# noah-aviel-dove/signals

Hardware: AMD Instinct MI355X
Metric: rendered Msamples/s (48 kHz, 256-sample blocks) (higher is better)
Workload: dtype f64; 1 GPU; C2: 1024-voice Fixed->Sine->LowPass->Gain->SumBus(stereo) per GPU, 48 kHz, 256-frame blocks, 4096 blocks per batch (f32 storage, f64 phase/recurrence); engine schedule = fused voice chain + bus: sig_fused_voice_bus (Sine->LowPass->Gain->SumBus in ONE launch, its voice tiles added in fixed order by the same kernel; no per-voice sample touches HBM); voices_per_gpu=1024, block_frames=256, start_position=0, parallelism=voices sharded 1024/GPU x1; single process, no collective, rccl_ranks=0

## Files before the change

### include/signals_amd.h

```cpp
#ifndef SIGNALS_AMD_H
#define SIGNALS_AMD_H

#include <stdint.h>

#ifdef __cplusplus
extern "C" {
#endif

#define SIG_ABI_VERSION 7

enum { SIG_F32 = 0, SIG_F64 = 1 };

enum { SIG_OSC_SINE = 0, SIG_OSC_SQUARE = 1, SIG_OSC_SAWTOOTH = 2, SIG_OSC_TRIANGLE = 3 };

enum { SIG_FILT_LOWPASS = 0, SIG_FILT_HIGHPASS = 1, SIG_FILT_BANDPASS = 2, SIG_FILT_BANDSTOP = 3 };

enum { SIG_EW_GAIN = 0, SIG_EW_MIX = 1, SIG_EW_RINGMOD = 2, SIG_EW_AMP = 3 };

enum { SIG_STATUS_BAD_CUTOFF = 1 };

int sig_abi_version(void);

int sig_osc_bank(int kind, int64_t position, int32_t rate, int64_t rows, int32_t voices,
                 const double* hertz, int32_t hertz_stride,
// ... 79 lines not shown

int sig_mix_matrix(int64_t rows, int32_t voices, const float* x, int64_t x_ld,
                   const float* matrix, float* out, int64_t out_ld, void* stream);

int sig_fused_osc_biquad(int osc_kind, int filt_type, int32_t rate, int64_t position,
                         int32_t block_frames, int32_t nblocks, int32_t context, int32_t voices,
                         const double* hertz, int32_t hertz_stride, const double* phase, int32_t phase_stride,
                         const double* cutoff, int32_t cutoff_stride,
                         const double* gain, int32_t gain_stride,
                         float* out, int64_t out_ld, int32_t* status, void* stream);

int sig_fused_osc_biquad_rows(int osc_kind, int filt_type, int32_t rate, int64_t position,
                              int32_t block_frames, int32_t nblocks, int32_t context, int32_t voices,
                              const double* hertz, int32_t hertz_stride, const double* phase, int32_t phase_stride,
                              const double* cutoff, int32_t cutoff_stride, int32_t cutoff_rows,
                              const double* gain, int32_t gain_stride, int32_t gain_rows,
                              float* out, int64_t out_ld, int32_t* status, void* stream);
int sig_fused_voice_bus_rows(int osc_kind, int filt_type, int32_t rate, int64_t position,
                             int32_t block_frames, int32_t nblocks, int32_t context, int32_t voices,
                             const double* hertz, int32_t hertz_stride, const double* phase, int32_t phase_stride,
                             const double* cutoff, int32_t cutoff_stride, int32_t cutoff_rows,
                             const double* gain, int32_t gain_stride, int32_t gain_rows,
                             const double* bus_gains, int64_t bus_gains_ld, int32_t bus_channels,
                             double* workspace, float* out, int64_t out_ld, int32_t* status, void* stream);

int sig_fused_osc_biquad_fm(int osc_kind, int filt_type, int32_t rate, int64_t position,
                            int32_t block_frames, int32_t nblocks, int32_t context, int32_t voices,
                            const double* hertz, int32_t hertz_stride, int32_t hertz_rows, const double* hertz_hist,
                            const double* phase, int32_t phase_stride, int32_t phase_rows, const double* phase_hist,
                            const double* cutoff, int32_t cutoff_stride, int32_t cutoff_rows,
                            const double* gain, int32_t gain_stride, int32_t gain_rows,
                            float* out, int64_t out_ld, int32_t* status, void* stream);
int sig_fused_voice_bus_fm(int osc_kind, int filt_type, int32_t rate, int64_t position,
                           int32_t block_frames, int32_t nblocks, int32_t context, int32_t voices,
                           const double* hertz, int32_t hertz_stride, int32_t hertz_rows, const double* hertz_hist,
                           const double* phase, int32_t phase_stride, int32_t phase_rows, const double* phase_hist,
                           const double* cutoff, int32_t cutoff_stride, int32_t cutoff_rows,
                           const double* gain, int32_t gain_stride, int32_t gain_rows,
                           const double* bus_gains, int64_t bus_gains_ld, int32_t bus_channels,
                           double* workspace, float* out, int64_t out_ld, int32_t* status, void* stream);

int sig_fused_osc_pair_biquad(int osc_kind, int osc2_kind, int pair_op, int filt_type, int32_t rate, int64_t position,
                              int32_t block_frames, int32_t nblocks, int32_t context, int32_t voices,
                              const double* hertz, int32_t hertz_stride, const double* phase, int32_t phase_stride,
                              const double* hertz2, int32_t hertz2_stride, const double* phase2, int32_t phase2_stride,
                              const double* mix, int32_t mix_stride,
                              const double* cutoff, int32_t cutoff_stride, int32_t cutoff_rows,
                              const double* gain, int32_t gain_stride, int32_t gain_rows,
                              float* out, int64_t out_ld, int32_t* status, void* stream);
int sig_fused_voice_pair_bus(int osc_kind, int osc2_kind, int pair_op, int filt_type, int32_t rate, int64_t position,
                             int32_t block_frames, int32_t nblocks, int32_t context, int32_t voices,
                             const double* hertz, int32_t hertz_stride, const double* phase, int32_t phase_stride,
                             const double* hertz2, int32_t hertz2_stride, const double* phase2, int32_t phase2_stride,
                             const double* mix, int32_t mix_stride,
                             const double* cutoff, int32_t cutoff_stride, int32_t cutoff_rows,
                             const double* gain, int32_t gain_stride, int32_t gain_rows,
                             const double* bus_gains, int64_t bus_gains_ld, int32_t bus_channels,
                             double* workspace, float* out, int64_t out_ld, int32_t* status, void* stream);

int sig_fused_osc_biquad_devpos(int osc_kind, int filt_type, int32_t rate, const int64_t* position_dev,
                                int32_t block_frames, int32_t nblocks, int32_t context, int32_t voices,
                                const double* hertz, int32_t hertz_stride, const double* phase, int32_t phase_stride,
                                const double* cutoff, int32_t cutoff_stride,
                                const double* gain, int32_t gain_stride,
                                float* out, int64_t out_ld, int32_t* status, void* stream);
int sig_advance_position(int64_t* position_dev, int64_t delta, void* stream);

enum { SIG_CTL_ROW = 0, SIG_CTL_OSC = 1, SIG_CTL_GAIN = 2, SIG_CTL_MIX = 3, SIG_CTL_RINGMOD = 4, SIG_CTL_AMP = 5,
       SIG_CTL_NOISE = 6, SIG_CTL_FILTER = 7 };
enum { SIG_CTL_MAX_REGS = 48, SIG_CTL_MAX_INS = 48 };
typedef struct {
    int32_t op;
    int32_t kind;
    int32_t a, b, c;
    int32_t dst;
    int32_t stride, rows;
    int32_t cols;
    int32_t reserved;
    const double* row;
} sig_ctl_ins;
typedef struct { int32_t reg; int32_t cols; double* out; double* front; } sig_ctl_out;
int sig_control_program(int32_t rate, int64_t position, int32_t step, int32_t nblocks, int32_t cols, int64_t front_position,
                        int64_t min_position,
                        const sig_ctl_ins* program, int32_t n_ins, const sig_ctl_out* outs, int32_t n_outs, void* stream);
int sig_control_program_windowed(int32_t rate, int64_t position, int32_t step, int32_t nblocks, int32_t cols, int64_t front_position,
                                 int64_t min_position,
                                 const sig_ctl_ins* program, int32_t n_ins, const sig_ctl_out* outs, int32_t n_outs, void* stream);

int sig_control_program_attach(const int32_t* description, int32_t n_words, const void* image, int32_t* handle);
int sig_control_program_attached(int32_t handle, int32_t rate, int64_t position, int32_t step, int32_t nblocks, int32_t cols,
                                 int64_t front_position, int64_t min_position,
                                 const sig_ctl_ins* program, int32_t n_ins, const sig_ctl_out* outs, int32_t n_outs, void* stream);

int sig_fused_osc_biquad_mix(int osc_kind, int filt_type, int32_t rate, int64_t position,
                             int32_t block_frames, int32_t nblocks, int32_t context, int32_t voices,
                             const double* hertz, int32_t hertz_stride, const double* phase, int32_t phase_stride,
                             const double* cutoff, int32_t cutoff_stride,
                             const double* gain, int32_t gain_stride,
                             const float* matrix, float* out, int64_t out_ld, int32_t* status, void* stream);

int64_t sig_fused_voice_bus_workspace(int32_t voices, int64_t rows, int32_t bus_channels);
int sig_fused_voice_bus_walk(int osc_kind, int filt_type, int32_t rate, int64_t position,
                             int32_t block_frames, int32_t nblocks, int32_t context, int32_t voices,
                             const double* hertz, int32_t hertz_stride, const double* phase, int32_t phase_stride,
                             const double* cutoff, int32_t cutoff_stride,
                             const double* gain, int32_t gain_stride,
                             const double* bus_gains, int64_t bus_gains_ld, int32_t bus_channels,
                             double* workspace, float* out, int64_t out_ld, int32_t* status, void* stream);
int64_t sig_fused_voice_consts_size(int32_t voices);
int sig_fused_voice_bus_prepared(int osc_kind, int filt_type, int32_t rate, int64_t position,
                                 int32_t block_frames, int32_t nblocks, int32_t context, int32_t voices,
                                 const double* hertz, int32_t hertz_stride, const double* phase, int32_t phase_stride,
                                 const double* cutoff, int32_t cutoff_stride,
                                 const double* gain, int32_t gain_stride,
                                 const double* bus_gains, int64_t bus_gains_ld, int32_t bus_channels,
                                 double* workspace, float* out, int64_t out_ld, int32_t* status, void* stream,
                                 double* consts, int32_t consts_ready);

typedef struct {
    int32_t osc_kind, filt_type, rate, block_frames, nblocks, context, voices;
    int32_t hertz_stride, phase_stride, cutoff_stride, gain_stride, bus_channels;
    const double* hertz; const double* phase; const double* cutoff; const double* gain; const double* bus_gains;
    int64_t bus_gains_ld, out_ld;
    double* workspace; int32_t* status; double* consts;
} sig_fused_voice_bus_call;
int sig_fused_voice_bus_bound(const sig_fused_voice_bus_call* call, int64_t position, float* out, int32_t consts_ready,
                              int32_t walk, void* stream);

int sig_fused_cascade_bus(int osc_kind, int filt1_type, int filt2_type, int32_t rate, int64_t position,
                          int64_t first_history_start, int32_t block_frames, int32_t nblocks, int32_t context,
                          int32_t voices,
                          const double* hertz, int32_t hertz_stride, const double* phase, int32_t phase_stride,
                          const double* cutoff1, int32_t cutoff1_stride, const double* cutoff2, int32_t cutoff2_stride,
                          const double* gain, int32_t gain_stride,
                          const double* const* adsr_params, const int32_t* adsr_strides,
                          const double* bus_gains, int64_t bus_gains_ld, int32_t bus_channels,
                          double* workspace, float* out, int64_t out_ld, int32_t* status, void* stream);
int sig_fused_cascade_geometry(int32_t voices, int32_t nblocks, int32_t* voices_per_lane, int32_t* blocks_per_lane);
int sig_fused_cascade_set_tuning(int32_t voices_per_lane, int32_t blocks_per_lane);

int64_t sig_latency_voice_bus_workspace(int32_t voices, int32_t block_frames, int32_t bus_channels);
int sig_latency_voice_bus(int filt_type, int32_t rate, int64_t position, int64_t* position_dev,
                          int32_t block_frames, int32_t context, int32_t voices,
                          const double* hertz, int32_t hertz_stride, const double* phase, int32_t phase_stride,
                          const double* cutoff, int32_t cutoff_stride,
                          const double* gain, int32_t gain_stride,
                          const double* bus_gains, int64_t bus_gains_ld, int32_t bus_channels,
                          double* workspace, float* out, int64_t out_ld, int32_t* status, void* stream);

int sig_fused_geometry(int32_t voices, int32_t block_frames, int32_t nblocks, int32_t context,
                       int32_t* voices_per_lane, int32_t* blocks_per_lane);
int sig_fused_voice_bus_plan(int osc_kind, int64_t position, int32_t voices, int32_t block_frames, int32_t nblocks,
                             int32_t context, int32_t* voices_per_lane, int32_t* blocks_per_lane, int32_t* closed_form);
int sig_fused_set_tuning(int32_t voices_per_lane, int32_t blocks_per_lane, int32_t closed_form, int32_t scan);
int sig_fused_voice_bus(int osc_kind, int filt_type, int32_t rate, int64_t position,
                        int32_t block_frames, int32_t nblocks, int32_t context, int32_t voices,
                        const double* hertz, int32_t hertz_stride, const double* phase, int32_t phase_stride,
                        const double* cutoff, int32_t cutoff_stride,
                        const double* gain, int32_t gain_stride,
                        const double* bus_gains, int64_t bus_gains_ld, int32_t bus_channels,
                        double* workspace, float* out, int64_t out_ld, int32_t* status, void* stream);

enum { SIG_VP_OSC = 0, SIG_VP_FILTER = 1, SIG_VP_GAIN = 2, SIG_VP_MUL = 3, SIG_VP_MIX = 4, SIG_VP_SAVE = 5, SIG_VP_LOAD = 6,
       SIG_VP_CONST = 7, SIG_VP_AMP = 8, SIG_VP_ADSR = 9, SIG_VP_NOISE = 10, SIG_VP_BAND = 11, SIG_VP_OSCPM = 12 };
enum { SIG_VP_MAX_INS = 32, SIG_VP_MAX_OSCS = 4, SIG_VP_MAX_PARAMS = 8, SIG_VP_MAX_FILTERS = 4, SIG_VP_MAX_TEMPS = 4, SIG_VP_MAX_HIST = 3 };
typedef struct { int32_t op, kind, a, b, c; } sig_vp_ins;
typedef struct { const double* ptr; int32_t col_stride; int32_t rows; } sig_vp_rows;
typedef struct {
    int32_t n_ins; sig_vp_ins ins[SIG_VP_MAX_INS];
    int32_t n_oscs; sig_vp_rows hertz[SIG_VP_MAX_OSCS], phase[SIG_VP_MAX_OSCS];
    int32_t n_params; sig_vp_rows params[SIG_VP_MAX_PARAMS];
    int32_t n_filters; sig_vp_rows cutoff[SIG_VP_MAX_FILTERS]; int32_t filter_type[SIG_VP_MAX_FILTERS];
    int32_t filter_level[SIG_VP_MAX_FILTERS];
    int32_t n_temps, depth;
    const double* adsr[6]; int32_t adsr_stride[6];
    uint64_t noise_seed[2];
} sig_voice_program_t;
int sig_voice_program(const sig_voice_program_t* program, int32_t rate, int64_t position, int32_t block_frames,
                      int32_t nblocks, int32_t context, int32_t voices, int32_t control_rows,
                      int32_t hist_blocks, const int64_t* hist_positions, int32_t blocks_before,
                      const double* bus_gains, int64_t bus_gains_ld, int32_t bus_channels,
                      double* workspace, float* out, int64_t out_ld, int32_t* status, void* stream);
int sig_voice_program_set_tuning(int32_t voices_per_lane, int32_t blocks_per_lane);
int sig_voice_program_geometry(int32_t voices, int32_t block_frames, int32_t nblocks, int32_t context, int32_t depth,
                               int32_t bus_channels, int32_t store_aligned, int32_t specialised,
                               int32_t* voices_per_lane, int32_t* blocks_per_lane);
int sig_voice_program_attach(const sig_voice_program_t* program, int32_t voices_per_lane, int32_t bus_channels, const void* image);
int sig_voice_program_detach_all(void);
int sig_voice_program_use_attached(int32_t on);
int64_t sig_voice_program_args_size(void);

#ifdef __cplusplus
}
#endif
#endif
```

### signals_amd/_native.py

```python
from __future__ import annotations

import ctypes
import pathlib

import torch

import os

LIB_PATH = pathlib.Path(os.environ.get('SIG_LIB_PATH') or pathlib.Path(__file__).resolve().parent / 'csrc' / 'libsignals_amd.so')

F32, F64 = 0, 1
OSC_KINDS = {'Sine': 0, 'Square': 1, 'Sawtooth': 2, 'Triangle': 3}
FILT_TYPES = {'lp': 0, 'hp': 1, 'bp': 2, 'bs': 3}
EW_OPS = {'Gain': 0, 'Mix': 1, 'RingMod': 2, 'Amp': 3}
STATUS_BAD_CUTOFF = 1
ABI_VERSION = 7
SINE_FAST_MAX_CYCLES = 2.0 ** 26

ADSR_PARAMS = ('attack', 'decay', 'sustain', 'release', 'gate_on', 'gate_off')


class NativeError(RuntimeError):
    """The HIP library is missing, was given a CPU tensor, or returned a hipError_t."""


class CtlIns(ctypes.Structure):
    _fields_ = [('op', ctypes.c_int32), ('kind', ctypes.c_int32), ('a', ctypes.c_int32), ('b', ctypes.c_int32), ('c', ctypes.c_int32),
                ('dst', ctypes.c_int32), ('stride', ctypes.c_int32), ('rows', ctypes.c_int32), ('cols', ctypes.c_int32),
                ('reserved', ctypes.c_int32), ('row', ctypes.c_void_p)]


class CtlOut(ctypes.Structure):
    _fields_ = [('reg', ctypes.c_int32), ('cols', ctypes.c_int32), ('out', ctypes.c_void_p), ('front', ctypes.c_void_p)]


CTL_OPS = {'Row': 0, 'Osc': 1, 'Gain': 2, 'Mix': 3, 'RingMod': 4, 'Amp': 5, 'Noise': 6, 'Filter': 7}
CTL_WINDOWED_OPS = (6, 7)
CTL_MAX_REGS, CTL_MAX_INS = 48, 48


VP_OPS = {'Osc': 0, 'Filter': 1, 'Gain': 2, 'Mul': 3, 'Mix': 4, 'Save': 5, 'Load': 6, 'Const': 7, 'Amp': 8, 'Adsr': 9, 'Noise': 10,
          'Band': 11, 'OscPM': 12}
VP_EXT_OPS = ('Amp', 'Adsr', 'Noise')
VP_MAX_INS, VP_MAX_OSCS, VP_MAX_PARAMS, VP_MAX_FILTERS, VP_MAX_TEMPS, VP_MAX_HIST = 32, 4, 8, 4, 4, 3


class VpIns(ctypes.Structure):
    _fields_ = [('op', ctypes.c_int32), ('kind', ctypes.c_int32), ('a', ctypes.c_int32), ('b', ctypes.c_int32), ('c', ctypes.c_int32)]


class VpRows(ctypes.Structure):
    _fields_ = [('ptr', ctypes.c_void_p), ('col_stride', ctypes.c_int32), ('rows', ctypes.c_int32)]


class VoiceProgramT(ctypes.Structure):
    _fields_ = [('n_ins', ctypes.c_int32), ('ins', VpIns * VP_MAX_INS),
                ('n_oscs', ctypes.c_int32), ('hertz', VpRows * VP_MAX_OSCS), ('phase', VpRows * VP_MAX_OSCS),
                ('n_params', ctypes.c_int32), ('params', VpRows * VP_MAX_PARAMS),
                ('n_filters', ctypes.c_int32), ('cutoff', VpRows * VP_MAX_FILTERS), ('filter_type', ctypes.c_int32 * VP_MAX_FILTERS),
                ('filter_level', ctypes.c_int32 * VP_MAX_FILTERS),
                ('n_temps', ctypes.c_int32), ('depth', ctypes.c_int32),
                ('adsr', ctypes.c_void_p * 6), ('adsr_stride', ctypes.c_int32 * 6), ('noise_seed', ctypes.c_uint64 * 2)]


class Operand(ctypes.Structure):
    _fields_ = [('ptr', ctypes.c_void_p), ('row_stride', ctypes.c_int64),
                ('col_stride', ctypes.c_int32), ('dtype', ctypes.c_int32),
                ('row_div', ctypes.c_int32), ('reserved', ctypes.c_int32)]


def _argtypes() -> dict:
    cint, i32, i64, u64, vp, dp = ctypes.c_int, ctypes.c_int32, ctypes.c_int64, ctypes.c_uint64, ctypes.c_void_p, ctypes.c_void_p
    p32, operand = ctypes.POINTER(i32), ctypes.POINTER(Operand)
    fused = [cint, cint, i32, i64, i32, i32, i32, i32]
    cold = [cint, i32, i64, i32, i32, i32, i32]
    rows4 = [dp, i32] * 4
    params = [dp, i32, i32] * 2
    env = [ctypes.POINTER(vp), p32]
    window = [vp, i64, i64]
    bus = [dp, i64, i32, vp]
    out = [vp, i64, vp, vp]
    program = [i32, i64, i32, i32, i32, i64, i64, vp, i32, vp, i32, vp]
    return {
        'sig_abi_version': [],
        'sig_osc_bank': [cint, i64, i32, i64, i32, dp, i32, dp, i32, vp, i32, i64, vp],
        'sig_osc_bank_mod': [cint, i64, i64, i32, i64, i32, i32, dp, i32, i64, dp, i32, i64, vp, i32, i64, vp],
        'sig_osc_bank_pm': [cint, i64, i64, i32, i64, i32, i32, dp, i32, i64, dp, i32, i64, dp, i32, i64,
                            vp, i32, i64, i32, vp, i32, i64, vp],
        'sig_biquad_coldstart': cold + [dp, i32, i32] + window + [vp, i64, i32, vp, vp],
        'sig_biquad_coldstart_env': cold + [dp, i32, i32] + env + window + out,
        'sig_biquad_coldstart_bus': cold + [dp, i32, i32] + env + window + bus + out,
        'sig_band_coldstart': cold + [dp, i32, dp, i32] + window + [vp, i64, i32, vp, vp],
        'sig_band_coldstart_blocks': cold + [dp, i32, dp, i32, i32] + window + [vp, i64, i32, vp, vp],
        'sig_elementwise': [cint, i64, i32, operand, operand, operand, vp, i64, i32, vp],
        'sig_sum_bus': [i64, i32, vp, i64, i32, dp, i64, i32, vp, i64, i32, vp],
        'sig_white_noise': [u64, i64, i64, i32, vp, i32, i64, vp],
        'sig_adsr': [i64, i32, i64, i32] + env + [vp, i32, i64, vp],
        'sig_adsr_apply': [i64, i32, i64, i32] + env + [vp, i64, vp, i64, vp],
        'sig_mix_matrix': [i64, i32, vp, i64, vp, vp, i64, vp],
        'sig_advance_position': [vp, i64, vp],
        'sig_fused_osc_biquad': fused + rows4 + out,
        'sig_fused_osc_biquad_devpos': [cint, cint, i32, vp, i32, i32, i32, i32] + rows4 + out,
        'sig_fused_osc_biquad_mix': fused + rows4 + [vp] + out,
        'sig_fused_osc_biquad_rows': fused + [dp, i32] * 2 + params + out,
        'sig_fused_osc_biquad_fm': fused + [dp, i32, i32, dp] * 2 + params + out,
        'sig_fused_osc_pair_biquad': [cint, cint] + fused + [dp, i32] * 5 + params + out,
        'sig_fused_voice_bus': fused + rows4 + bus + out,
        'sig_fused_voice_bus_walk': fused + rows4 + bus + out,
        'sig_fused_voice_bus_prepared': fused + rows4 + bus + out + [vp, i32],
        'sig_fused_voice_bus_bound': [vp, i64, vp, i32, i32, vp],
        'sig_fused_voice_bus_rows': fused + [dp, i32] * 2 + params + bus + out,
        'sig_fused_voice_bus_fm': fused + [dp, i32, i32, dp] * 2 + params + bus + out,
        'sig_fused_voice_pair_bus': [cint, cint] + fused + [dp, i32] * 5 + params + bus + out,
        'sig_fused_voice_bus_workspace': [i32, i64, i32],
        'sig_fused_voice_consts_size': [i32],
        'sig_fused_voice_bus_plan': [cint, i64, i32, i32, i32, i32, p32, p32, p32],
        'sig_fused_geometry': [i32, i32, i32, i32, p32, p32],
        'sig_fused_set_tuning': [i32, i32, i32, i32],
        'sig_fused_cascade_bus': [cint, cint, cint, i32, i64, i64, i32, i32, i32, i32] + [dp, i32] * 5 + env + bus + out,
        'sig_fused_cascade_geometry': [i32, i32, p32, p32],
        'sig_fused_cascade_set_tuning': [i32, i32],
        'sig_latency_voice_bus': [cint, i32, i64, vp, i32, i32, i32] + rows4 + bus + out,
        'sig_latency_voice_bus_workspace': [i32, i32, i32],
        'sig_control_program': program,
        'sig_control_program_windowed': program,
        'sig_control_program_attach': [p32, i32, ctypes.c_char_p, p32],
        'sig_control_program_attached': [i32] + program,
        'sig_voice_program': [ctypes.POINTER(VoiceProgramT), i32, i64, i32, i32, i32, i32, i32, i32, ctypes.POINTER(i64), i32] + bus + out,
        'sig_voice_program_set_tuning': [i32, i32],
        'sig_voice_program_geometry': [i32, i32, i32, i32, i32, i32, i32, i32, p32, p32],
        'sig_voice_program_args_size': [],
        'sig_voice_program_attach': [ctypes.POINTER(VoiceProgramT), i32, i32, ctypes.c_char_p],
        'sig_voice_program_detach_all': [],
        'sig_voice_program_use_attached': [i32],
    }


_ARGTYPES = _argtypes()
_RETURNS_INT64 = ('sig_fused_voice_bus_workspace', 'sig_fused_voice_consts_size', 'sig_latency_voice_bus_workspace',
                  'sig_voice_program_args_size')
EXPORTS = tuple(_ARGTYPES)

_lib = None


def lib() -> ctypes.CDLL:
    global _lib
    if _lib is None:
        if not LIB_PATH.exists():
            raise NativeError(f'{LIB_PATH} not built: run `python -c "import __graft_entry__ as g; g.build()"` '
                              f'(signals_amd/csrc/build.sh).  There is no CPU fallback.')
        L = ctypes.CDLL(str(LIB_PATH))
        for name, argtypes in _ARGTYPES.items():
            entry = getattr(L, name)
            entry.restype = ctypes.c_int64 if name in _RETURNS_INT64 else ctypes.c_int
            entry.argtypes = argtypes
        if L.sig_abi_version() != ABI_VERSION:
            raise NativeError('libsignals_amd.so ABI version mismatch')
        _lib = L
    return _lib


def _check(err: int, what: str) -> None:
    if err != 0:
        raise NativeError(f'{what} failed: hipError_t {err}')


def _dt(t: torch.Tensor) -> int:
    if t.dtype == torch.float32:
        return F32
    if t.dtype == torch.float64:
        return F64
    raise NativeError(f'unsupported buffer dtype {t.dtype}')


def _gpu(*tensors: torch.Tensor) -> None:
    for t in tensors:
        if t is not None and not t.is_cuda:
            raise NativeError('HIP kernels need tensors resident on an MI355X (got a CPU tensor); no CPU fallback')


_raw_stream = getattr(torch._C, '_cuda_getCurrentRawStream', None)


def _stream(t: torch.Tensor) -> int:
    if _raw_stream is not None:
        return _raw_stream(t.device.index)
    return torch.cuda.current_stream(t.device).cuda_stream


def current_stream_handle(device_index: int) -> int:
    if _raw_stream is not None:
        return _raw_stream(device_index)
    return torch.cuda.current_stream(device_index).cuda_stream


def _ctrl_row(t: torch.Tensor | None, what: str):
    if t is None:
        return None, 0
    if t.dtype != torch.float64 or t.dim() != 2 or t.shape[0] != 1 or (t.shape[1] > 1 and t.stride(1) != 1):
        raise NativeError(f'{what}: control rows are contiguous float64 (1,V) or (1,1), got {tuple(t.shape)} {t.dtype}')
    return t.data_ptr(), (0 if t.shape[1] == 1 else 1)


def _audio(t: torch.Tensor, what: str) -> None:
    if t.dim() != 2 or (t.shape[1] > 1 and t.stride(1) != 1):
        raise NativeError(f'{what}: audio buffers are 2-D with contiguous channels, got strides {t.stride()}')


def _ctrl_rows(t: torch.Tensor | None, what: str):
    if t is None:
        return None, 0, 0, 1
    if t.dtype != torch.float64 or t.dim() != 2 or (t.shape[1] > 1 and t.stride(1) != 1):
        raise NativeError(f'{what}: control rows are float64 (R,V) or (R,1) with contiguous channels, got '
                          f'{tuple(t.shape)} {t.dtype}')
    return t.data_ptr(), (0 if t.shape[1] == 1 else 1), (0 if t.shape[0] == 1 else t.stride(0)), t.shape[0]


def _ptr(t: torch.Tensor | None):
    return None if t is None else t.data_ptr()


def _voice_rows(voices: int, *pairs, form=_ctrl_row) -> list:
    flat = []
    for row, name in pairs:
        if row is not None and row.shape[1] not in (1, voices):
            raise NativeError(f'{name} has {row.shape[1]} channels for {voices} voices')
        flat.extend(form(row, name))
    return flat


def _bus_gains(gains: torch.Tensor | None, bus: int, voices: int):
    if gains is None:
        if bus != 1:
            raise NativeError('a bus without gains is mono')
        return None, 0
    if gains.dtype != torch.float64 or gains.shape != (bus, voices) or gains.stride(1) != 1:
        raise NativeError(f'bus gains must be float64 ({bus},{voices}), got {tuple(gains.shape)} {gains.dtype}')
    return gains.data_ptr(), gains.stride(0)


def _envelope(rows: dict | None, voices: int, into: tuple | None = None):
    if rows is None:
        return None, None
    ptrs, strides = into or ((ctypes.c_void_p * 6)(), (ctypes.c_int32 * 6)())
    flat = _voice_rows(voices, *((rows[name], name) for name in ADSR_PARAMS))
    for i in range(6):
        ptrs[i], strides[i] = flat[2 * i], flat[2 * i + 1]
    return ptrs, strides


def _bus_workspace(workspace: torch.Tensor | None, voices: int, rows: int, bus: int, device=None) -> torch.Tensor:
    need = lib().sig_fused_voice_bus_workspace(voices, rows, bus)
    fits = workspace is not None and workspace.numel() * workspace.element_size() >= need
    if device is None and not (fits and workspace.dtype == torch.float64):
        raise NativeError('fused bus workspace too small')
    return workspace if fits else torch.empty(need // 8, dtype=torch.float64, device=device)


def _history_input(buf: torch.Tensor, history: int, voices: int, out: torch.Tensor, block_frames: int, nblocks: int, what: str) -> int:
    rows = out.shape[0]
    if rows != block_frames * nblocks or buf.shape[0] != history + rows or buf.shape[1] != voices or buf.dtype != out.dtype:
        raise NativeError(f'{what} shapes: in {tuple(buf.shape)} {buf.dtype} history {history} out {tuple(out.shape)} {out.dtype} '
                          f'blocks {nblocks}x{block_frames}')
    return buf.data_ptr() + history * buf.stride(0) * buf.element_size()


def _parameter_rows(rows: int, rows_per_param: int, *counts) -> int:
    if max(n for n, _ in counts) == 1:
# ... 123 lines not shown
    _audio(out, 'noise out')
    _check(lib().sig_white_noise(seed, position, out.shape[0], out.shape[1], out.data_ptr(), _dt(out),
                                 out.stride(0), _stream(out)), 'sig_white_noise')
    return out


def adsr(position: int, rate: int, rows: dict, out: torch.Tensor) -> torch.Tensor:
    _gpu(out, *rows.values())
    _audio(out, 'adsr out')
    _check(lib().sig_adsr(position, rate, out.shape[0], out.shape[1], *_envelope(rows, out.shape[1]), out.data_ptr(), _dt(out),
                          out.stride(0), _stream(out)), 'sig_adsr')
    return out


def mix_matrix(x: torch.Tensor, matrix: torch.Tensor, out: torch.Tensor) -> torch.Tensor:
    _gpu(x, matrix, out)
    _audio(x, 'mix_matrix in')
    _audio(out, 'mix_matrix out')
    if x.dtype != torch.float32 or out.dtype != torch.float32 or matrix.dtype != torch.float32:
        raise NativeError('mix_matrix is float32 in / float32 out')
    if matrix.shape != (64, 64) or not matrix.is_contiguous() or x.shape != out.shape or x.shape[1] % 64:
        raise NativeError(f'mix_matrix shapes: x {tuple(x.shape)} matrix {tuple(matrix.shape)} out {tuple(out.shape)}')
    _check(lib().sig_mix_matrix(x.shape[0], x.shape[1], x.data_ptr(), x.stride(0), matrix.data_ptr(),
                                out.data_ptr(), out.stride(0), _stream(out)), 'sig_mix_matrix')
    return out


def fused_osc_biquad(kind: str, btype: str, rate: int, position, block_frames: int, nblocks: int, context: int,
                     hertz: torch.Tensor, phase: torch.Tensor | None, cutoff: torch.Tensor,
                     gain: torch.Tensor | None, out: torch.Tensor, status: torch.Tensor | None = None) -> torch.Tensor:
    _gpu(hertz, phase, cutoff, gain, out, status)
    _audio(out, 'fused out')
    rows, voices = out.shape
    if out.dtype != torch.float32 or rows != block_frames * nblocks:
        raise NativeError(f'fused out must be float32 ({block_frames * nblocks}, V), got {tuple(out.shape)} {out.dtype}')
    ptrs = _voice_rows(voices, (hertz, 'hertz'), (phase, 'phase'), (cutoff, 'cutoff'), (gain, 'gain'))
    entry, name = lib().sig_fused_osc_biquad, 'sig_fused_osc_biquad'
    if isinstance(position, torch.Tensor):
        entry, name, position = lib().sig_fused_osc_biquad_devpos, 'sig_fused_osc_biquad_devpos', _device_position(position)
    _check(entry(OSC_KINDS[kind], FILT_TYPES[btype], rate, position, block_frames, nblocks, context, voices, *ptrs,
                 out.data_ptr(), out.stride(0), _ptr(status), _stream(out)), name)
    return out


def _device_position(position: torch.Tensor) -> int:
    if position.dtype != torch.int64 or position.numel() != 1 or not position.is_cuda:
        raise NativeError('device position must be a one-element int64 GPU tensor')
    return position.data_ptr()


def biquad_coldstart_bus(btype: str, rate: int, position: int, block_frames: int, nblocks: int, context: int,
                         cutoff: torch.Tensor, buf: torch.Tensor, history: int, bus_gains: torch.Tensor | None,
                         out: torch.Tensor, envelope: dict | None = None, workspace: torch.Tensor | None = None,
                         status: torch.Tensor | None = None) -> torch.Tensor:
    _gpu(cutoff, buf, out, status, bus_gains, *(envelope or {}).values())
    _audio(buf, 'biquad bus in')
    _audio(out, 'biquad bus out')
    rows, bus = out.shape
    voices = buf.shape[1]
    if out.dtype != torch.float32:
        raise NativeError(f'biquad bus out must be float32, got {out.dtype}')
    in_ptr = _history_input(buf, history, voices, out, block_frames, nblocks, 'biquad bus')
    if cutoff.dtype != torch.float64 or cutoff.shape[1] not in (1, voices) or cutoff.shape[0] not in (1, nblocks) \
            or not cutoff.is_contiguous():
        raise NativeError(f'cutoff must be contiguous float64 (1|{nblocks}, 1|{voices}), got {tuple(cutoff.shape)} {cutoff.dtype}')
    workspace = _bus_workspace(workspace, voices, rows, bus, out.device)
    _check(lib().sig_biquad_coldstart_bus(FILT_TYPES[btype], rate, position, block_frames, nblocks, context, voices,
                                          cutoff.data_ptr(), 0 if cutoff.shape[1] == 1 else 1, cutoff.shape[0],
                                          *_envelope(envelope, voices), in_ptr, buf.stride(0), history,
                                          *_bus_gains(bus_gains, bus, voices), bus, workspace.data_ptr(),
                                          out.data_ptr(), out.stride(0), _ptr(status), _stream(out)),
           'sig_biquad_coldstart_bus')
    return out


def latency_voice_bus_workspace(voices: int, block_frames: int, bus_channels: int, device) -> torch.Tensor:
    return torch.zeros(lib().sig_latency_voice_bus_workspace(voices, block_frames, bus_channels) // 8, dtype=torch.float64,
                       device=device)


def latency_voice_bus(btype: str, rate: int, position, block_frames: int, context: int, voices: int,
                      hertz: torch.Tensor, phase: torch.Tensor | None, cutoff: torch.Tensor, gain: torch.Tensor | None,
                      bus_gains: torch.Tensor | None, out: torch.Tensor, workspace: torch.Tensor,
                      status: torch.Tensor | None = None) -> torch.Tensor:
    _gpu(out)
    _audio(out, 'latency bus out')
    rows, bus = out.shape
    if out.dtype != torch.float32 or rows != block_frames:
        raise NativeError(f'latency bus out must be float32 ({block_frames}, C), got {tuple(out.shape)} {out.dtype}')
    call = LatencyVoiceBusCall(btype, rate, block_frames, context, voices, hertz, phase, cutoff, gain, bus_gains, bus, workspace,
                               status)
    pos_int, pos_dev = position, None
    if isinstance(position, torch.Tensor):
        pos_int, pos_dev = 0, _device_position(position)
    _check(call._fn(*call._head, pos_int, pos_dev, *call._mid, out.data_ptr(), out.stride(0), call._status, _stream(out)),
           'sig_latency_voice_bus')
    return out


class LatencyVoiceBusCall:

    def __init__(self, btype: str, rate: int, block_frames: int, context: int, voices: int,
                 hertz: torch.Tensor, phase: torch.Tensor | None, cutoff: torch.Tensor, gain: torch.Tensor | None,
                 bus_gains: torch.Tensor | None, bus_channels: int, workspace: torch.Tensor,
                 status: torch.Tensor | None = None):
        _gpu(hertz, phase, cutoff, gain, bus_gains, workspace, status)
        need = lib().sig_latency_voice_bus_workspace(voices, block_frames, bus_channels)
        if workspace.dtype != torch.float64 or workspace.numel() * 8 < need:
            raise NativeError(f'latency workspace needs {need} bytes of float64 (latency_voice_bus_workspace)')
        ptrs = _voice_rows(voices, (hertz, 'hertz'), (phase, 'phase'), (cutoff, 'cutoff'), (gain, 'gain'))
        gp, gld = _bus_gains(bus_gains, bus_channels, voices)
        self._keep = (hertz, phase, cutoff, gain, bus_gains, workspace, status)
        self._fn = lib().sig_latency_voice_bus
        self._head = (FILT_TYPES[btype], rate)
        self._mid = (block_frames, context, voices, *ptrs, gp, gld, bus_channels, workspace.data_ptr())
        self._status = _ptr(status)
        self.shape = (block_frames, bus_channels)
        self.device = workspace.device

    def __call__(self, position: int, out: torch.Tensor) -> torch.Tensor:
        err = self._fn(*self._head, position, None, *self._mid, out.data_ptr(), self.shape[1], self._status, _stream(out))
        if err:
            raise NativeError(f'sig_latency_voice_bus failed: hipError_t {err}')
        return out


class FusedVoiceBusCallT(ctypes.Structure):
    _fields_ = [(n, ctypes.c_int32) for n in ('osc_kind', 'filt_type', 'rate', 'block_frames', 'nblocks', 'context', 'voices',
                                              'hertz_stride', 'phase_stride', 'cutoff_stride', 'gain_stride', 'bus_channels')] + \
               [(n, ctypes.c_void_p) for n in ('hertz', 'phase', 'cutoff', 'gain', 'bus_gains')] + \
               [('bus_gains_ld', ctypes.c_int64), ('out_ld', ctypes.c_int64), ('workspace', ctypes.c_void_p), ('status', ctypes.c_void_p),
                ('consts', ctypes.c_void_p)]


class FusedVoiceBusCall:

    def __init__(self, kind: str, btype: str, rate: int, block_frames: int, nblocks: int, context: int, voices: int,
                 hertz: torch.Tensor, phase: torch.Tensor | None, cutoff: torch.Tensor, gain: torch.Tensor | None,
                 bus_gains: torch.Tensor | None, bus_channels: int, workspace: torch.Tensor, status: torch.Tensor | None,
                 consts: torch.Tensor):
        _gpu(hertz, phase, cutoff, gain, bus_gains, workspace, status, consts)
        rows = block_frames * nblocks
        hp, hs, pp, ps, cp, cs, gp_, gs = _voice_rows(voices, (hertz, 'hertz'), (phase, 'phase'), (cutoff, 'cutoff'), (gain, 'gain'))
        gp, gld = _bus_gains(bus_gains, bus_channels, voices)
        _bus_workspace(workspace, voices, rows, bus_channels)
        self._keep = (hertz, phase, cutoff, gain, bus_gains, workspace, status, consts)
        self.shape = (rows, bus_channels)
        self._block = FusedVoiceBusCallT(OSC_KINDS[kind], FILT_TYPES[btype], rate, block_frames, nblocks, context, voices, hs, ps, cs, gs,
                                         bus_channels, hp, pp, cp, gp_, gp, gld, bus_channels, workspace.data_ptr(), _ptr(status),
                                         _consts(consts, voices))
        self._block_ref = ctypes.byref(self._block)
        self._bound = lib().sig_fused_voice_bus_bound

    def __call__(self, position: int, out: torch.Tensor, consts_ready: bool, walk: bool = False, stream: int | None = None) -> torch.Tensor:
        s = _stream(out) if stream is None else stream
        err = self._bound(self._block_ref, position, out.data_ptr(), 1 if consts_ready else 0, 1 if walk else 0, s)
        if err:
            raise NativeError(f'sig_fused_voice_bus failed: hipError_t {err}')
        return out


def _consts(consts: torch.Tensor, voices: int) -> int:
    if consts.dtype != torch.float64 or consts.numel() * 8 < lib().sig_fused_voice_consts_size(voices):
        raise NativeError('consts must be float64 of sig_fused_voice_consts_size(voices) bytes')
    return consts.data_ptr()


def fused_geometry(voices: int, block_frames: int, nblocks: int, context: int) -> tuple[int, int]:
    vpt, span = ctypes.c_int32(), ctypes.c_int32()
    _check(lib().sig_fused_geometry(voices, block_frames, nblocks, context, ctypes.byref(vpt), ctypes.byref(span)),
           'sig_fused_geometry')
    return vpt.value, span.value


def _param_rows(t: torch.Tensor | None, what: str, voices: int, nblocks: int):
    if t is None:
        return None, 0, 1
    if t.dtype != torch.float64 or t.dim() != 2 or not t.is_contiguous() or t.shape[1] not in (1, voices) or t.shape[0] not in (1, nblocks):
        raise NativeError(f'{what}: per-block parameters are contiguous float64 (1|{nblocks}, 1|{voices}), got {tuple(t.shape)} {t.dtype}')
    return t.data_ptr(), (0 if t.shape[1] == 1 else 1), t.shape[0]


def fused_rows(kind: str, btype: str, rate: int, position: int, block_frames: int, nblocks: int, context: int, voices: int,
               hertz: torch.Tensor, phase: torch.Tensor | None, cutoff: torch.Tensor, gain: torch.Tensor | None,
               out: torch.Tensor, bus_gains: torch.Tensor | None = None, bus: bool = False,
               workspace: torch.Tensor | None = None, status: torch.Tensor | None = None,
               pair: tuple | None = None, hertz_hist: torch.Tensor | None = None,
               phase_hist: torch.Tensor | None = None) -> torch.Tensor:
    _gpu(hertz, phase, cutoff, gain, out, bus_gains, workspace, status, hertz_hist, phase_hist,
         *((pair[2], pair[3], pair[4]) if pair else ()))
    _audio(out, 'fused rows out')
    rows = out.shape[0]
    if out.dtype != torch.float32 or rows != block_frames * nblocks:
        raise NativeError(f'fused rows out must be float32 ({block_frames * nblocks}, .), got {tuple(out.shape)} {out.dtype}')
    kinds = (OSC_KINDS[kind], FILT_TYPES[btype])
    if hertz_hist is not None or phase_hist is not None or hertz.shape[0] > 1 or (phase is not None and phase.shape[0] > 1):
        if pair is not None:
            raise NativeError('block-rate FM and a second oscillator: no fused entry point')
        names = ('sig_fused_osc_biquad_fm', 'sig_fused_voice_bus_fm')
        source = []
        for t, front, what in ((hertz, hertz_hist, 'hertz'), (phase, phase_hist, 'phase')):
            ptr, stride, count = _param_rows(t, what, voices, nblocks)
            if t is not None and not (front is None and count == 1):
                if front is None or front.dtype != torch.float64 or tuple(front.shape) != (1, t.shape[1]) or not front.is_contiguous():
                    raise NativeError(f'{what}_hist: the row in front of the launch is float64 (1, {t.shape[1]})')
            source += [ptr, stride, count, _ptr(front) if t is not None else None]
    else:
        names = ('sig_fused_osc_biquad_rows', 'sig_fused_voice_bus_rows')
        source = _voice_rows(voices, (hertz, 'hertz'), (phase, 'phase'))
        if pair is not None:
            op, kind2, hertz2, phase2, mixrow = pair
            names = ('sig_fused_osc_pair_biquad', 'sig_fused_voice_pair_bus')
            kinds = (OSC_KINDS[kind], OSC_KINDS[kind2], {'Mix': 1, 'RingMod': 2}[op], FILT_TYPES[btype])
            source += _voice_rows(voices, (hertz2, 'hertz2'), (phase2, 'phase2'), (mixrow, 'mix'))
    sink = ()
    if bus:
        C = out.shape[1]
        workspace = _bus_workspace(workspace, voices, rows, C, out.device)
        sink = (*_bus_gains(bus_gains, C, voices), C, workspace.data_ptr())
    elif out.shape[1] != voices:
        raise NativeError(f'fused rows out has {out.shape[1]} channels for {voices} voices')
    name = names[1 if bus else 0]
    _check(getattr(lib(), name)(*kinds, rate, position, block_frames, nblocks, context, voices, *source,
                                *_param_rows(cutoff, 'cutoff', voices, nblocks), *_param_rows(gain, 'gain', voices, nblocks),
                                *sink, out.data_ptr(), out.stride(0), _ptr(status), _stream(out)), name)
    return out


def fused_cascade_bus(kind: str, btype1: str, btype2: str, rate: int, position: int, first_history_start: int,
                      block_frames: int, nblocks: int, context: int, voices: int,
                      hertz: torch.Tensor, phase: torch.Tensor | None, cutoff1: torch.Tensor, cutoff2: torch.Tensor,
                      gain: torch.Tensor | None, envelope: dict | None, bus_gains: torch.Tensor | None, out: torch.Tensor,
                      workspace: torch.Tensor | None = None, status: torch.Tensor | None = None) -> torch.Tensor:
    _gpu(hertz, phase, cutoff1, cutoff2, gain, bus_gains, out, workspace, status, *(envelope or {}).values())
    _audio(out, 'fused cascade out')
    rows, bus = out.shape
    if out.dtype != torch.float32 or rows != block_frames * nblocks:
        raise NativeError(f'fused cascade out must be float32 ({block_frames * nblocks}, C), got {tuple(out.shape)} {out.dtype}')
    ptrs = _voice_rows(voices, (hertz, 'hertz'), (phase, 'phase'), (cutoff1, 'cutoff1'), (cutoff2, 'cutoff2'), (gain, 'gain'))
    workspace = _bus_workspace(workspace, voices, rows, bus, out.device)
    _check(lib().sig_fused_cascade_bus(OSC_KINDS[kind], FILT_TYPES[btype1], FILT_TYPES[btype2], rate, position,
                                       first_history_start, block_frames, nblocks, context, voices, *ptrs,
                                       *_envelope(envelope, voices), *_bus_gains(bus_gains, bus, voices), bus,
                                       workspace.data_ptr(), out.data_ptr(), out.stride(0), _ptr(status), _stream(out)),
           'sig_fused_cascade_bus')
    return out


def fused_cascade_geometry(voices: int, nblocks: int) -> tuple[int, int]:
    vpt, span = ctypes.c_int32(), ctypes.c_int32()
    _check(lib().sig_fused_cascade_geometry(voices, nblocks, ctypes.byref(vpt), ctypes.byref(span)), 'sig_fused_cascade_geometry')
    return vpt.value, span.value


def set_fused_cascade_tuning(voices_per_lane: int = 0, blocks_per_lane: int = 0) -> None:
    _check(lib().sig_fused_cascade_set_tuning(voices_per_lane, blocks_per_lane), 'sig_fused_cascade_set_tuning')


def fused_cascade_model(voices: int, block_frames: int, nblocks: int, context: int = 100, bus_channels: int = 1,
                        osc_ops: float = 5.0, envelope: bool = True) -> dict:
    vpt, span = fused_cascade_geometry(voices, nblocks)
    n, c = block_frames, context
    walked = (span * n + n + c) / (span * n)
    products = max(c, 1).bit_length() - 1 + bin(max(c, 1)).count('1')
    restart = 8.0 * products + 6.0
    ops = (osc_ops + 4.0) * walked + 4.0 * (1.0 + c / (span * n)) + (bus_channels if envelope else 0.0) + bus_channels \
        + 17.0 * bus_channels / (16 * vpt) + restart * (2 * (span - 1) + 1) / (span * n)
    return {'f64_ops_per_voice_sample': ops, 'voices_per_lane': vpt, 'blocks_per_lane': span,
            'rows_walked_per_output_row': walked}


def upload_structs(items: list) -> torch.Tensor:
    arr = (type(items[0]) * len(items))(*items)
    host = torch.frombuffer(bytearray(bytes(arr)), dtype=torch.uint8)
    return host.to(runtime_device())


def runtime_device():
    from . import runtime
    return runtime.device()


def control_program(rate: int, position: int, step: int, nblocks: int, cols: int, program: torch.Tensor, n_ins: int,
                    outs: torch.Tensor, n_outs: int, front_position: int = -1, min_position: int = 0, windowed: bool = False) -> None:
    _gpu(program, outs)
    entry = lib().sig_control_program_windowed if windowed else lib().sig_control_program
    _check(entry(rate, position, step, nblocks, cols, front_position, min_position, program.data_ptr(), n_ins,
                                     outs.data_ptr(), n_outs, _stream(program)), 'sig_control_program')


def control_program_description(ins: list, outs: list) -> list:
    words = [len(ins), len(outs)]
    for x in ins:
        words += [x.op, x.kind, x.a, x.b, x.c, x.dst, (1 if x.cols > 1 else 0) | (2 if x.reserved else 0)]
    for o in outs:
        words += [o.reg, 1 if o.cols > 1 else 0]
    return words


def control_program_attach(description: list, image: bytes) -> int:
    arr = (ctypes.c_int32 * len(description))(*description)
    handle = ctypes.c_int32(0)
    _check(lib().sig_control_program_attach(arr, len(description), image, ctypes.byref(handle)), 'sig_control_program_attach')
    return handle.value


def control_program_attached(handle: int, rate: int, position: int, step: int, nblocks: int, cols: int, program: torch.Tensor,
                             n_ins: int, outs: torch.Tensor, n_outs: int, front_position: int = -1, min_position: int = 0) -> None:
    _gpu(program, outs)
    _check(lib().sig_control_program_attached(handle, rate, position, step, nblocks, cols, front_position, min_position,
                                              program.data_ptr(), n_ins, outs.data_ptr(), n_outs, _stream(program)),
           'sig_control_program_attached')


def fused_voice_bus_plan(kind: str, position: int, voices: int, block_frames: int, nblocks: int, context: int) -> dict:
    vpt, span, closed = ctypes.c_int32(), ctypes.c_int32(), ctypes.c_int32()
    _check(lib().sig_fused_voice_bus_plan(OSC_KINDS[kind], position, voices, block_frames, nblocks, context,
                                          ctypes.byref(vpt), ctypes.byref(span), ctypes.byref(closed)),
           'sig_fused_voice_bus_plan')
    kernel = f'fused_steady_bus_kernel<{vpt.value}, C>' if closed.value else f'fused_walk_kernel<{kind}, {vpt.value}, gain, C>'
    return {'voices_per_lane': vpt.value, 'blocks_per_lane': span.value, 'closed_form': bool(closed.value), 'kernel': kernel}


def set_fused_tuning(voices_per_lane: int = 0, blocks_per_lane: int = 0, closed_form: int = -1, scan: int = -1) -> None:
    _check(lib().sig_fused_set_tuning(voices_per_lane, blocks_per_lane, closed_form, scan), 'sig_fused_set_tuning')


def fused_osc_biquad_mix(kind: str, btype: str, rate: int, position: int, block_frames: int, nblocks: int, context: int,
                         hertz: torch.Tensor, phase: torch.Tensor | None, cutoff: torch.Tensor,
                         gain: torch.Tensor | None, matrix: torch.Tensor, out: torch.Tensor,
                         status: torch.Tensor | None = None) -> torch.Tensor:
    _gpu(hertz, phase, cutoff, gain, matrix, out, status)
    _audio(out, 'fused mix out')
    rows, voices = out.shape
    if out.dtype != torch.float32 or rows != block_frames * nblocks or voices % 64:
        raise NativeError(f'fused mix out must be float32 ({block_frames * nblocks}, 64*g), got {tuple(out.shape)} {out.dtype}')
    if matrix.dtype != torch.float32 or tuple(matrix.shape) != (64, 64) or not matrix.is_contiguous():
        raise NativeError(f'mix matrix must be contiguous float32 (64, 64), got {tuple(matrix.shape)} {matrix.dtype}')
    ptrs = _voice_rows(voices, (hertz, 'hertz'), (phase, 'phase'), (cutoff, 'cutoff'), (gain, 'gain'))
    _check(lib().sig_fused_osc_biquad_mix(OSC_KINDS[kind], FILT_TYPES[btype], rate, position, block_frames, nblocks, context,
                                          voices, *ptrs, matrix.data_ptr(), out.data_ptr(), out.stride(0), _ptr(status),
                                          _stream(out)), 'sig_fused_osc_biquad_mix')
    return out


def advance_position(position: torch.Tensor, delta: int) -> None:
    _gpu(position)
    _check(lib().sig_advance_position(position.data_ptr(), delta, _stream(position)), 'sig_advance_position')


def fused_voice_bus(kind: str, btype: str, rate: int, position: int, block_frames: int, nblocks: int, context: int,
                    voices: int, hertz: torch.Tensor, phase: torch.Tensor | None, cutoff: torch.Tensor,
                    gain: torch.Tensor | None, bus_gains: torch.Tensor | None, out: torch.Tensor,
                    workspace: torch.Tensor | None = None, status: torch.Tensor | None = None,
                    consts: torch.Tensor | None = None, consts_ready: bool = False, walk: bool = False) -> torch.Tensor:
    _gpu(hertz, phase, cutoff, gain, bus_gains, out, status, consts)
    _audio(out, 'fused bus out')
    rows, bus = out.shape
    if out.dtype != torch.float32 or rows != block_frames * nblocks:
        raise NativeError(f'fused bus out must be float32 ({block_frames * nblocks}, C), got {tuple(out.shape)} {out.dtype}')
    ptrs = _voice_rows(voices, (hertz, 'hertz'), (phase, 'phase'), (cutoff, 'cutoff'), (gain, 'gain'))
    workspace = _bus_workspace(workspace, voices, rows, bus, out.device)
    entry, name, tail = lib().sig_fused_voice_bus, 'sig_fused_voice_bus', ()
    if walk:
        entry, name = lib().sig_fused_voice_bus_walk, 'sig_fused_voice_bus_walk'
    elif consts is not None:
        entry, name = lib().sig_fused_voice_bus_prepared, 'sig_fused_voice_bus_prepared'
        tail = (_consts(consts, voices), 1 if consts_ready else 0)
    _check(entry(OSC_KINDS[kind], FILT_TYPES[btype], rate, position, block_frames, nblocks, context, voices, *ptrs,
                 *_bus_gains(bus_gains, bus, voices), bus, workspace.data_ptr(), out.data_ptr(), out.stride(0), _ptr(status),
                 _stream(out), *tail), name)
    return out


def band_coldstart(btype: str, rate: int, position: int, block_frames: int, nblocks: int, context: int,
                   low: torch.Tensor, high: torch.Tensor, buf: torch.Tensor, history: int, out: torch.Tensor,
                   status: torch.Tensor | None = None) -> torch.Tensor:
    return _band_coldstart(False, btype, rate, position, block_frames, nblocks, context, low, high, buf, history, out, status)


def band_coldstart_blocks(btype: str, rate: int, position: int, block_frames: int, nblocks: int, context: int,
                          low: torch.Tensor, high: torch.Tensor, buf: torch.Tensor, history: int, out: torch.Tensor,
                          status: torch.Tensor | None = None) -> torch.Tensor:
    return _band_coldstart(True, btype, rate, position, block_frames, nblocks, context, low, high, buf, history, out, status)


def _band_coldstart(per_block: bool, btype, rate, position, block_frames, nblocks, context, low, high, buf, history, out, status):
    _gpu(low, high, buf, out, status)
    _audio(buf, 'band in')
    _audio(out, 'band out')
    voices = out.shape[1]
    in_ptr = _history_input(buf, history, voices, out, block_frames, nblocks, 'band')
    blocks = max(low.shape[0], high.shape[0])
    edges = []
    for row, name in ((low, 'low'), (high, 'high')):
        if row.shape[1] != voices and voices != 1:
            raise IndexError(f'index {row.shape[1]} is out of bounds for axis 1 with size {row.shape[1]}')
        if per_block:
            if row.dtype != torch.float64 or row.dim() != 2 or not row.is_contiguous():
                raise NativeError(f'{name} must be a contiguous float64 2-D tensor')
            if row.shape[0] not in (1, nblocks):
                raise NativeError(f'{name} has {row.shape[0]} rows for {nblocks} blocks')
            if row.shape[0] != blocks:
                row = row.expand(blocks, row.shape[1]).contiguous()
        edges.append((row, name))
    if per_block:
        name, entry = 'sig_band_coldstart_blocks', lib().sig_band_coldstart_blocks
        ptrs = _voice_rows(voices, *edges, form=lambda t, what: _ctrl_rows(t, what)[:2]) + [blocks]
    else:
        name, entry = 'sig_band_coldstart', lib().sig_band_coldstart
        ptrs = _voice_rows(voices, *edges)
    _check(entry(FILT_TYPES[btype], rate, position, block_frames, nblocks, context, voices, *ptrs, in_ptr, buf.stride(0), history,
                 out.data_ptr(), out.stride(0), _dt(out), _ptr(status), _stream(out)), name)
    return out


def adsr_apply(position: int, rate: int, rows: dict, x: torch.Tensor, out: torch.Tensor) -> torch.Tensor:
    _gpu(x, out, *rows.values())
    _audio(x, 'adsr_apply in')
    _audio(out, 'adsr_apply out')
    if x.dtype != torch.float32 or out.dtype != torch.float32 or x.shape != out.shape:
        raise NativeError(f'adsr_apply is float32 (rows, V) in and out, got {tuple(x.shape)} {x.dtype} -> {tuple(out.shape)} {out.dtype}')
    _check(lib().sig_adsr_apply(position, rate, out.shape[0], out.shape[1], *_envelope(rows, out.shape[1]), x.data_ptr(),
                                x.stride(0), out.data_ptr(), out.stride(0), _stream(out)), 'sig_adsr_apply')
    return out


def _vp_rows(t: torch.Tensor | None, what: str, voices: int, control_rows: int) -> VpRows:
    if t is None:
        return VpRows(None, 0, 1)
    if (t.dtype != torch.float64 or t.dim() != 2 or not t.is_contiguous() or t.shape[1] not in (1, voices)
            or t.shape[0] not in (1, control_rows)):
        raise NativeError(f'{what}: rows of a voice program are contiguous float64 (1|{control_rows}, 1|{voices}), got {tuple(t.shape)} {t.dtype}')
    return VpRows(t.data_ptr(), 0 if t.shape[1] == 1 else 1, t.shape[0])


def _program_struct(code: list) -> VoiceProgramT:
    P = VoiceProgramT()
    P.n_ins = len(code)
    for k, (op, kind, a, b, c) in enumerate(code):
        P.ins[k] = VpIns(VP_OPS[op], kind, a, b, c)
    return P


def voice_program(code: list, oscs: list, params: list, filters: list, n_temps: int, depth: int, rate: int, position: int,
                  block_frames: int, nblocks: int, context: int, voices: int, control_rows: int, hist_positions: list,
                  out: torch.Tensor, bus_gains: torch.Tensor | None = None, bus: bool = False,
                  adsr: dict | None = None, noise_seeds: tuple = (0, 0), workspace: torch.Tensor | None = None,
                  status: torch.Tensor | None = None, blocks_before: int = 0) -> torch.Tensor:
    tensors = [t for pair in oscs for t in pair] + list(params) + [f[0] for f in filters] + list((adsr or {}).values())
    _gpu(out, bus_gains, workspace, status, *tensors)
    _audio(out, 'voice program out')
    rows = block_frames * nblocks
    if out.dtype != torch.float32 or out.shape[0] != rows:
        raise NativeError(f'voice program out must be float32 ({rows}, .), got {tuple(out.shape)} {out.dtype}')
    if len(code) > VP_MAX_INS or len(oscs) > VP_MAX_OSCS or len(params) > VP_MAX_PARAMS or len(filters) > VP_MAX_FILTERS \
            or n_temps > VP_MAX_TEMPS or len(hist_positions) > VP_MAX_HIST:
        raise NativeError('voice program larger than the machine')
    P = _program_struct(code)
    P.n_oscs = len(oscs)
    for k, (hz, ph) in enumerate(oscs):
        P.hertz[k] = _vp_rows(hz, 'hertz', voices, control_rows)
        P.phase[k] = _vp_rows(ph, 'phase', voices, control_rows)
    P.n_params = len(params)
    for k, t in enumerate(params):
        P.params[k] = _vp_rows(t, 'parameter', voices, control_rows)
    P.n_filters = len(filters)
    for k, (cut, btype, level) in enumerate(filters):
        if cut.shape[1] != voices and voices != 1:
            raise IndexError(f'index {cut.shape[1]} is out of bounds for axis 1 with size {cut.shape[1]}')
        P.cutoff[k] = _vp_rows(cut, 'cutoff', voices, control_rows)
        P.filter_type[k] = FILT_TYPES[btype]
        P.filter_level[k] = level
    P.n_temps, P.depth = n_temps, depth
    _envelope(adsr, voices, into=(P.adsr, P.adsr_stride))
    P.noise_seed[0], P.noise_seed[1] = noise_seeds
    hist = (ctypes.c_int64 * max(1, len(hist_positions)))(*hist_positions)
    C = 0
    gp, gld = None, 0
    if bus:
        C = out.shape[1]
        gp, gld = _bus_gains(bus_gains, C, voices)
        workspace = _bus_workspace(workspace, voices, rows, C, out.device)
    elif out.shape[1] != voices:
        raise NativeError(f'voice program out has {out.shape[1]} channels for {voices} voices')
    _check(lib().sig_voice_program(ctypes.byref(P), rate, position, block_frames, nblocks, context, voices, control_rows,
                                   len(hist_positions), hist, blocks_before, gp, gld, C,
                                   _ptr(workspace), out.data_ptr(), out.stride(0), _ptr(status), _stream(out)), 'sig_voice_program')
    return out


def voice_program_words(code: list) -> list:
    return [VP_OPS[op] | (kind << 5) | (a << 8) | (b << 12) | (c << 16) for op, kind, a, b, c in code]


def voice_program_geometry(voices: int, block_frames: int, nblocks: int, context: int, depth: int, bus_channels: int,
                           store_aligned: int, specialised: bool = False) -> tuple:
    vpt, span = ctypes.c_int32(0), ctypes.c_int32(0)
    _check(lib().sig_voice_program_geometry(voices, block_frames, nblocks, context, depth, bus_channels, int(store_aligned),
                                            1 if specialised else 0, ctypes.byref(vpt), ctypes.byref(span)), 'sig_voice_program_geometry')
    return vpt.value, span.value


def voice_program_attach(code: list, n_oscs: int, n_params: int, n_filters: int, n_temps: int, voices_per_lane: int,
                         bus_channels: int, image: bytes) -> None:
    P = _program_struct(code)
    P.n_oscs, P.n_params, P.n_filters, P.n_temps = n_oscs, n_params, n_filters, n_temps
    _check(lib().sig_voice_program_attach(ctypes.byref(P), voices_per_lane, bus_channels, image), 'sig_voice_program_attach')


def voice_program_detach_all() -> None:
    _check(lib().sig_voice_program_detach_all(), 'sig_voice_program_detach_all')


def voice_program_use_attached(on: bool) -> None:
    _check(lib().sig_voice_program_use_attached(1 if on else 0), 'sig_voice_program_use_attached')


def set_voice_program_tuning(voices_per_lane: int = 0, blocks_per_lane: int = 0) -> None:
    _check(lib().sig_voice_program_set_tuning(voices_per_lane, blocks_per_lane), 'sig_voice_program_set_tuning')
```

### signals_amd/csrc/fused_voice.hip

```cpp
#include <cstdlib>
#include <type_traits>

#include "sig_biquad.h"
#include "sig_bus_tile.h"
#include "sig_mix_tile.h"
#include "sig_osc.h"
#include "sig_steady.h"

#if defined(SIG_TUNE_SINE_ONLY)
#define SIG_FUSED_SPLIT 0
#define SIG_FUSED_HERE_SINE 1
#define SIG_FUSED_HERE_OTHERS 0
#elif defined(SIG_FUSED_PART_B)
#define SIG_FUSED_SPLIT 1
#define SIG_FUSED_HERE_SINE 0
#define SIG_FUSED_HERE_OTHERS 1
#else
#define SIG_FUSED_SPLIT 1
#define SIG_FUSED_HERE_SINE 1
#define SIG_FUSED_HERE_OTHERS 0
#endif

namespace {

// ... 236 lines not shown
        };
        int done = 0;
        constexpr bool GROUPED = FAST || KIND != SIG_OSC_SINE || ROWS;
        if (!OUT || !BUS) {
            constexpr int U = GROUPED ? 4 : 1;
            for (; done + U <= count; done += U) {
                ensure(U);
#pragma unroll
                for (int k = 0; k < U; ++k) {
                    double x[VPT], y[VPT];
                    gen(x, k);
                    chains(x, y, w0, w1, warm_tag);
                    if (OUT) to_out(y, out_row + done + k);
                }
                n_cur += U;
            }
            for (; done < count; ++done) {
                double x[VPT], y[VPT];
                ensure(1);
                gen(x, 0);
                chains(x, y, w0, w1, warm_tag);
                if (OUT) to_out(y, out_row + done);
                ++n_cur;
            }
            return;
        }
        auto single = [&]() {
            double x[VPT], y[VPT];
            ensure(1);
            gen(x, 0);
            chains(x, y, w0, w1, warm_tag);
            to_tile(y, stage.slot);
            ++n_cur; ++done;
            stage.advance();
        };
        while (stage.staged != 0 && done < count) single();
        double pend[4];
        int64_t pend_row = 0;
        bool have = false;
        for (; GROUPED && done + R <= count; done += R) {
            ensure(R);
            double acc[kPairs];
#pragma unroll
            for (int k = 0; k < R; ++k) {
                double x[VPT], y[VPT];
                gen(x, k);
                chains(x, y, w0, w1, warm_tag);
                to_tile(y, acc + k * CC, 1);
#pragma unroll
                for (int g = 0; g < kPairs / 4; ++g)
                    if (4 * g + 3 < (k + 1) * CC && 4 * g + 3 >= k * CC)
                        folded.fold4(g, acc[4 * g], acc[4 * g + 1], acc[4 * g + 2], acc[4 * g + 3]);
                if (k + 1 == R / 2 && have) folded.finish(pend, pend_row, R);
            }
            n_cur += R;
            folded.issue(pend);
            pend_row = stage.first; stage.first += R; have = true;
        }
        if (have) folded.finish(pend, pend_row, R);
        while (done < count) single();
    };
    auto walk_any = [&](int count, int64_t out_row, double (&w0)[VPT], double (&w1)[VPT], auto out_tag, auto warm_tag, int64_t blk) {
        if constexpr (ROWS) {
            if (a.pair_op != 0) {
                if (KIND == SIG_OSC_SINE && fast) walk(count, out_row, w0, w1, out_tag, warm_tag, std::true_type{}, std::true_type{}, blk);
                else walk(count, out_row, w0, w1, out_tag, warm_tag, std::false_type{}, std::true_type{}, blk);
                return;
            }
        }
        if (KIND == SIG_OSC_SINE && fast) walk(count, out_row, w0, w1, out_tag, warm_tag, std::true_type{}, std::false_type{}, blk);
        else walk(count, out_row, w0, w1, out_tag, warm_tag, std::false_type{}, std::false_type{}, blk);
    };

    walk_any(c0, 0, z0, z1, std::false_type{}, std::false_type{}, b_first - 1);
    for (int bi = 0; bi < nb; ++bi) {
        const int64_t orow = (b_first + bi) * a.N;
        const int tail = (bi + 1 < nb) ? a.ctx : 0;
        walk_any(a.N - tail, orow, z0, z1, std::true_type{}, std::false_type{}, b_first + bi);
        if (tail) {
            double w0[VPT], w1[VPT];
#pragma unroll
            for (int i = 0; i < VPT; ++i) { w0[i] = 0.0; w1[i] = 0.0; }
            if constexpr (ROWS) {
                if (a.cutoff_rows > 1 || a.gain_rows > 1) {
                    design_block(b_first + bi + 1, wna1, wna2, [&](int ch, int i, double w) { wwt[ch][i] = w; });
                } else {
#pragma unroll
                    for (int i = 0; i < VPT; ++i) {
                        wna1[i] = na1[i]; wna2[i] = na2[i];
#pragma unroll
                        for (int ch = 0; ch < CC; ++ch) wwt[ch][i] = wt[ch][i];
                    }
                }
            }
            walk_any(tail, orow + a.N - tail, w0, w1, std::true_type{}, std::true_type{}, b_first + bi);
#pragma unroll
            for (int i = 0; i < VPT; ++i) { z0[i] = w0[i]; z1[i] = w1[i]; }
            if constexpr (ROWS) {
#pragma unroll
                for (int i = 0; i < VPT; ++i) {
                    na1[i] = wna1[i]; na2[i] = wna2[i];
#pragma unroll
                    for (int ch = 0; ch < CC; ++ch) wt[ch][i] = wwt[ch][i];
                }
            }
        }
    }
    if (BUS && stage.staged) stage.now();
    if constexpr (MIX) sink.finish();
}

template <int KIND, int VPT, bool GAIN, int C, bool ROWS = false>
__global__ __launch_bounds__(256) __attribute__((amdgpu_waves_per_eu(Occ<VPT>::lo, Occ<VPT>::hi)))
void fused_walk_kernel(FusedArgs a, BusArgs bus)
{
    constexpr bool BUS = C > 0, MIX = C < 0;
    __shared__ __attribute__((aligned(16))) double lds[(BUS || MIX) ? 4 : 1][BUS ? kPairs * kTileStride : (MIX ? sig_mix::kTileRows * sig_mix::kLdsStride / 2 : 1)];
    const int lane = threadIdx.x & 63;
    const int wave = __builtin_amdgcn_readfirstlane(threadIdx.x >> 6);
    walk_wave<KIND, VPT, GAIN, C, ROWS>(a, bus, lds[(BUS || MIX) ? wave : 0], lane, wave);
    if constexpr (BUS) {
        if (bus.out) sig_bus::sum_tiles_in_workgroup<C>(bus.partials, a.voice_tiles, bus.rows, a.span, a.K, a.N, bus.out, bus.out_ld, lane, wave);
    }
}

enum { SC_NA1, SC_NA2, SC_SCALE, SC_K2C, SC_ST, SC_CT, SC_HRE, SC_HIM, SC_ND, SC_T, SC_T0 = SC_T + 4, kSteadyConsts = SC_T0 + 4 };

__device__ __forceinline__ bool steady_wave(const FusedArgs& a, int v0, int vpt, int64_t p0, int nb) {
    const double q_first = (double)p0 / a.rate, q_last = (double)(p0 + (int64_t)nb * a.N - 1) / a.rate;
    bool ok = true;
    for (int i = 0; i < vpt; ++i) {
        const int v = (v0 + i < a.voices) ? v0 + i : ((v0 < a.voices) ? v0 : 0);
        ok &= steady_voice_ok(a.hertz[(int64_t)v * a.hs], a.phase ? a.phase[(int64_t)v * a.ps] : 0.0, a.rate,
                              a.steady_consts[(int64_t)SC_ST * a.voices + v], q_first, q_last);
    }
    return __all(ok);
}

template <bool GAIN>
__global__ __launch_bounds__(256) void steady_prep_kernel(FusedArgs a, double* __restrict__ consts)
{
    const int v = blockIdx.x * blockDim.x + threadIdx.x;
    if (v >= a.voices) return;
    const SteadyVoice c = steady_constants<GAIN>(a, v);
    if (!c.ok && a.status) atomicOr(a.status, SIG_STATUS_BAD_CUTOFF);
    auto put = [&](int k, double x) { consts[(int64_t)k * a.voices + v] = x; };
    put(SC_NA1, c.na1); put(SC_NA2, c.na2); put(SC_SCALE, c.scale);
    put(SC_K2C, c.k2c); put(SC_ST, c.st); put(SC_CT, c.ct);
    put(SC_HRE, c.hre); put(SC_HIM, c.him); put(SC_ND, c.nd);
    put(SC_T + 0, c.T.a); put(SC_T + 1, c.T.b); put(SC_T + 2, c.T.c); put(SC_T + 3, c.T.d);
    put(SC_T0 + 0, c.T0.a); put(SC_T0 + 1, c.T0.b); put(SC_T0 + 2, c.T0.c); put(SC_T0 + 3, c.T0.d);
}

template <int VPT, int C>
__device__ __forceinline__ void steady_fallback_span(const FusedArgs& a, const BusArgs& bus, double* tile, int lane, int vt,
                                                  int64_t b_first, int nb, int v0)
{
    const int vc = (v0 < a.voices) ? v0 : 0;
    const double* sc = a.steady_consts;
    const double s2 = (a.type == SIG_FILT_LOWPASS) ? 2.0 : -2.0;
    sig_bus::PipelinedTile<C> stage(tile, lane, bus.partials + (int64_t)vt * bus.rows * C, b_first * a.N);
    for (int i = 0; i < VPT; ++i)
        if (v0 + i < a.voices && a.status && sc[(int64_t)SC_NA1 * a.voices + v0 + i] != sc[(int64_t)SC_NA1 * a.voices + v0 + i])
            atomicOr(a.status, SIG_STATUS_BAD_CUTOFF);
#pragma unroll 1
    for (int bi = 0; bi < nb; ++bi) {
        const int64_t p_b = a.position + (b_first + bi) * a.N;
        const int c = (int)((p_b < (int64_t)a.ctx) ? p_b : (int64_t)a.ctx);
        double z0[VPT], z1[VPT];
#pragma unroll
        for (int i = 0; i < VPT; ++i) z0[i] = z1[i] = 0.0;
#pragma unroll 1
        for (int r = -c; r < a.N; ++r) {
            const double q = (double)(p_b + r) / a.rate;
            double acc[C];
#pragma unroll
            for (int ch = 0; ch < C; ++ch) acc[ch] = 0.0;
#pragma unroll
            for (int i = 0; i < VPT; ++i) {
                const bool live = v0 + i < a.voices;
                const int v = live ? v0 + i : vc;
                const double t = q * a.hertz[(int64_t)v * a.hs] + (a.phase ? a.phase[(int64_t)v * a.ps] : 0.0);
                const double x = (double)sig_osc::osc_sine_f32(t);
                double na1 = sc[(int64_t)SC_NA1 * a.voices + v], na2 = sc[(int64_t)SC_NA2 * a.voices + v];
                double scale = live ? sc[(int64_t)SC_SCALE * a.voices + v] : 0.0;
                if (a.cutoff_rows > 1) {
                    Biquad qd;
                    design_butter2(a.type, a.cutoff[(b_first + bi) * (int64_t)(a.cs ? a.voices : 1) + (int64_t)v * a.cs], a.rate, qd);
                    na1 = -qd.a1; na2 = -qd.a2;
                    scale = live ? qd.b0 : 0.0;
                    if (a.gain && a.gain_rows == 1) scale *= a.gain[(int64_t)v * a.gs];
                }
                const double y = x + z0[i];
                z0[i] = fma(na1, y, fma(s2, x, z1[i]));
                z1[i] = fma(na2, y, x);
                if (a.gain_rows > 1) scale *= a.gain[(b_first + bi) * (int64_t)(a.gs ? a.voices : 1) + (int64_t)v * a.gs];
#pragma unroll
                for (int ch = 0; ch < C; ++ch) acc[ch] = fma(bus.pan ? bus.pan[ch * bus.pan_ld + v] * scale : scale, y, acc[ch]);
            }
            if (r >= 0) {
#pragma unroll
                for (int ch = 0; ch < C; ++ch) stage.slot[ch * kTileStride] = acc[ch];
                stage.advance();
            }
        }
    }
    if (stage.staged) stage.now();
}


template <int VPT> struct SteadyVariants {
    static constexpr int count = (VPT >= 8) ? 7 : (VPT == 4) ? 4 : (VPT == 2) ? 3 : 2;
    static constexpr int at(int k) {
        constexpr int v8[7] = {8, 6, 4, 3, 2, 1, 0}, v4[4] = {4, 2, 1, 0}, v2[3] = {2, 1, 0}, v1[2] = {1, 0};
        return (VPT >= 8) ? v8[k] : (VPT == 4) ? v4[k] : (VPT == 2) ? v2[k] : v1[k];
    }
};

#ifndef SIG_STEADY_OCC8
#define SIG_STEADY_OCC8 1
#endif
#ifndef SIG_STEADY_AUTO16
#define SIG_STEADY_AUTO16 0
#endif
#ifndef SIG_STEADY_OCC16
#define SIG_STEADY_OCC16 1
#endif
template <int VPT> struct SteadyOcc { static constexpr int waves = (VPT == 16) ? SIG_STEADY_OCC16 : (VPT == 8) ? SIG_STEADY_OCC8 : 2; };

template <int VPT, int C, bool GROWS, bool CROWS = false>
__device__ __forceinline__ void steady_bus_wave(const FusedArgs& a, const BusArgs& bus, double* tile, int lane, int wave, double* osc_store = nullptr)
{
    constexpr bool OSC_LDS = CROWS && VPT >= 8;
    constexpr int R = kPairs / C;
    constexpr int LC = SteadyVariants<VPT>::at(0);
    static_assert(R % 2 == 0, "the two-term recurrence rotates two registers per voice: row groups are even");
    const int64_t item = (int64_t)blockIdx.x * 4 + wave;
    const int vt = (int)(item % a.voice_tiles);
    const int64_t b_first = (item / a.voice_tiles) * a.span;
    if (b_first >= a.K) return;
    const int nb = (int)((a.K - b_first < (int64_t)a.span) ? a.K - b_first : (int64_t)a.span);
    const int v0 = (vt * SIG_WAVE + lane) * VPT;
    const int vc = (v0 < a.voices) ? v0 : 0;
    const int64_t p0 = a.position + b_first * a.N;
    if (!steady_wave(a, v0, VPT, p0, nb)) {
        steady_fallback_span<VPT, C>(a, bus, tile, lane, vt, b_first, nb, v0);
        return;
    }
    const double* sc = a.steady_consts;

    double na1[LC], na2[LC], k2c[VPT], ya[VPT], yb[VPT], wt[C][VPT];
    int nd_total[VPT];
    const double q_first = (double)p0 / a.rate;
#pragma unroll
    for (int i = 0; i < VPT; ++i) {
        const bool live = v0 + i < a.voices;
        const int v = live ? v0 + i : vc;
        auto cst = [&](int k) { return sc[(int64_t)k * a.voices + v]; };
        const double na1_i = cst(SC_NA1);
        if (i < LC) { na1[i < LC ? i : 0] = na1_i; na2[i < LC ? i : 0] = cst(SC_NA2); }
        k2c[i] = cst(SC_K2C);
        if (live && na1_i != na1_i && a.status) atomicOr(a.status, SIG_STATUS_BAD_CUTOFF);
        const double scale = cst(SC_SCALE);
#pragma unroll
        for (int ch = 0; ch < C; ++ch)
            wt[ch][i] = live ? (bus.pan ? bus.pan[ch * bus.pan_ld + v] * scale : scale) : 0.0;
        const double hz = a.hertz[(int64_t)v * a.hs], ph = a.phase ? a.phase[(int64_t)v * a.ps] : 0.0;
        const double t_first = q_first * hz + ph;
        const double f0 = t_first - rint(t_first);
        const double ur = sin2pi(f0 + 0.25), ui = sin2pi(f0);
        const double hre = cst(SC_HRE), him = cst(SC_HIM);
        const double wr = fma(hre, ur, -(him * ui)), wi = fma(hre, ui, him * ur);
        yb[i] = wi;
        ya[i] = fma(wi, cst(SC_CT), -(wr * cst(SC_ST)));
        const double nd = cst(SC_ND);
        nd_total[i] = (live && nd < (double)kNeverDrops) ? (int)nd : (live ? kNeverDrops : 0);
    }
#pragma unroll
    for (int d = 1; d < SIG_WAVE; d <<= 1) {
        int other[VPT];
#pragma unroll
        for (int i = 0; i < VPT; ++i) other[i] = __shfl_xor(nd_total[i], d, SIG_WAVE);
#pragma unroll
        for (int i = 0; i < VPT; ++i) nd_total[i] = (other[i] > nd_total[i]) ? other[i] : nd_total[i];
    }
#pragma unroll
    for (int i = 0; i < VPT; ++i) nd_total[i] = __builtin_amdgcn_readfirstlane(nd_total[i]);

    double* dstp = bus.partials + (int64_t)vt * bus.rows * C;
    sig_bus::PipelinedTile<C> stage(tile, lane, dstp, b_first * a.N);

    if constexpr (LC < VPT) {
        const int c_min = (b_first == 0 && a.position < (int64_t)a.ctx) ? (int)a.position : a.ctx;
        bool capped = true;
#pragma unroll
        for (int i = LC; i < VPT; ++i) capped &= nd_total[i] <= c_min;
        if (!capped) {
            steady_fallback_span<VPT, C>(a, bus, tile, lane, vt, b_first, nb, v0);
            return;
        }
    }
    [[maybe_unused]] OscPart osc[(CROWS && !OSC_LDS) ? VPT : 1];
    auto osc_slot = [&](int field, int i) -> double& { return osc_store[((size_t)field * VPT + i) * SIG_WAVE + lane]; };
    if constexpr (CROWS) {
#pragma unroll
        for (int i = 0; i < VPT; ++i) {
            const int v = (v0 + i < a.voices) ? v0 + i : vc;
            const OscPart made = steady_osc_part(a.type, a.hertz[(int64_t)v * a.hs], a.rate, a.ctx);
            if constexpr (OSC_LDS) {
                osc_slot(0, i) = made.ct; osc_slot(1, i) = made.st; osc_slot(2, i) = made.beta; osc_slot(3, i) = made.enr; osc_slot(4, i) = made.eni;
            } else {
                osc[i] = made;
            }
        }
    }
    double z0h[LC], z1h[LC];
    auto row = [&](double* sums, int sums_stride, auto m_tag, auto odd_tag) {
        constexpr int M = decltype(m_tag)::value;
        constexpr bool ODD = decltype(odd_tag)::value;
        double y[VPT];
#pragma unroll
        for (int i = 0; i < VPT; ++i) {
            const double ys = ODD ? ya[i] : yb[i];
            if (ODD) yb[i] = fma(k2c[i], ya[i], -yb[i]);
            else ya[i] = fma(k2c[i], yb[i], -ya[i]);
            if (i < M) {
                const int j = i < LC ? i : 0;
                y[i] = ys + z0h[j];
                const double yh = z0h[j];
                z0h[j] = fma(na1[j], yh, z1h[j]);
                z1h[j] = na2[j] * yh;
            } else {
                y[i] = ys;
            }
        }
#pragma unroll
        for (int ch = 0; ch < C; ++ch) {
            double acc = 0.0;
#pragma unroll
            for (int i = 0; i < VPT; ++i) acc = fma(wt[ch][i], y[i], acc);
            sums[ch * sums_stride] = acc;
        }
    };
    sig_bus::FoldedGroup<C> folded(tile, lane, dstp);
    double pend[4];
    int64_t pend_row = 0;
    bool have = false;
    auto rows2 = [&](double* sums, auto m_tag) {
        constexpr int M = decltype(m_tag)::value;
        double y0[VPT], y1[VPT];
#pragma unroll
        for (int i = 0; i < VPT; ++i) {
            y0[i] = yb[i];
            ya[i] = fma(k2c[i], yb[i], -ya[i]);
            y1[i] = ya[i];
            yb[i] = fma(k2c[i], ya[i], -yb[i]);
            if (i < M) {
                const int j = i < LC ? i : 0;
                const double h0 = z0h[j];
                y0[i] += h0;
                const double h1 = fma(na1[j], h0, z1h[j]);
                y1[i] += h1;
                z0h[j] = fma(na1[j], h1, na2[j] * h0);
                z1h[j] = na2[j] * h1;
            }
        }
        double acc0[C], acc1[C];
#pragma unroll
        for (int ch = 0; ch < C; ++ch) { acc0[ch] = 0.0; acc1[ch] = 0.0; }
#pragma unroll
        for (int i = 0; i < VPT; ++i) {
#pragma unroll
            for (int ch = 0; ch < C; ++ch) {
                acc0[ch] = fma(wt[ch][i], y0[i], acc0[ch]);
                acc1[ch] = fma(wt[ch][i], y1[i], acc1[ch]);
            }
        }
#pragma unroll
        for (int ch = 0; ch < C; ++ch) { sums[ch] = acc0[ch]; sums[C + ch] = acc1[ch]; }
    };
    auto group = [&](auto m_tag) {
        double acc[kPairs];
#pragma unroll
        for (int k = 0; k < R; k += 2) {
            rows2(acc + k * C, m_tag);
#pragma unroll
            for (int q = 0; q < kPairs / 4; ++q)
                if (4 * q + 3 < (k + 2) * C && 4 * q + 3 >= k * C)
                    folded.fold4(q, acc[4 * q], acc[4 * q + 1], acc[4 * q + 2], acc[4 * q + 3]);
            if (k + 2 == R / 2 && have) folded.finish(pend, pend_row, R);
        }
        folded.issue(pend);
        pend_row = stage.first; stage.first += R; have = true;
    };
    using Variants = SteadyVariants<VPT>;

    for (int bi = 0; bi < nb; ++bi) {
        if constexpr (GROWS && !CROWS) {
#pragma unroll
            for (int i = 0; i < VPT; ++i) {
                const bool live = v0 + i < a.voices;
                const int v = live ? v0 + i : vc;
                const double scale = sc[(int64_t)SC_SCALE * a.voices + v] * a.gain[(b_first + bi) * (int64_t)(a.gs ? a.voices : 1) + (int64_t)v * a.gs];
#pragma unroll
                for (int ch = 0; ch < C; ++ch) wt[ch][i] = live ? (bus.pan ? bus.pan[ch * bus.pan_ld + v] * scale : scale) : 0.0;
            }
        }
        const bool first = (b_first + bi == 0);
        const int tk = first ? SC_T0 : SC_T;
        const int c = first ? (int)((a.position < (int64_t)a.ctx) ? a.position : (int64_t)a.ctx) : a.ctx;
        if constexpr (CROWS) {
            const int64_t blk = b_first + bi;
            const double q_b = (double)(p0 + (int64_t)bi * a.N) / a.rate;
            double cut_i[VPT], gain_i[VPT];
#pragma unroll
            for (int i = 0; i < VPT; ++i) {
                const int v = (v0 + i < a.voices) ? v0 + i : vc;
                cut_i[i] = a.cutoff[(a.cutoff_rows > 1 ? blk * (int64_t)(a.cs ? a.voices : 1) : 0) + (int64_t)v * a.cs];
                gain_i[i] = a.gain ? a.gain[(a.gain_rows > 1 ? blk * (int64_t)(a.gs ? a.voices : 1) : 0) + (int64_t)v * a.gs] : 1.0;
            }
#pragma unroll
            for (int i = 0; i < VPT; ++i) {
                const bool live = v0 + i < a.voices;
                const int v = live ? v0 + i : vc;
                const double cutoff = cut_i[i], gain = gain_i[i];
                const double hz_v = a.hertz[(int64_t)v * a.hs], ph_v = a.phase ? a.phase[(int64_t)v * a.ps] : 0.0;
                OscPart op;
                if constexpr (OSC_LDS) op = OscPart{osc_slot(0, i), osc_slot(1, i), osc_slot(2, i), osc_slot(3, i), osc_slot(4, i)};
                else op = osc[i];
                if (__builtin_expect(c != a.ctx, 0)) op = steady_osc_part(a.type, hz_v, a.rate, c);
                const double ct_i = op.ct, st_i = op.st;
                const BlockVoice cv = steady_block_constants(a.type, a.rate, cutoff, gain, op, c);
                if (i < LC) { na1[i < LC ? i : 0] = cv.na1; na2[i < LC ? i : 0] = cv.na2; }
                if (live && !cv.ok && a.status) atomicOr(a.status, SIG_STATUS_BAD_CUTOFF);
#pragma unroll
                for (int ch = 0; ch < C; ++ch) wt[ch][i] = live ? (bus.pan ? bus.pan[ch * bus.pan_ld + v] * cv.scale : cv.scale) : 0.0;
                const double t_first = q_b * hz_v + ph_v;
                const double f0 = t_first - rint(t_first);
                const double ur = sin2pi(f0 + 0.25), ui = sin2pi(f0);
                const double wr = fma(cv.hre, ur, -(cv.him * ui)), wi = fma(cv.hre, ui, cv.him * ur);
                yb[i] = wi;
                ya[i] = fma(wi, ct_i, -(wr * st_i));
                if (i < LC) {
                    const double dss = fma(k2c[i], yb[i], -ya[i]) - yb[i];
                    z0h[i < LC ? i : 0] = fma(cv.T.a, yb[i], cv.T.b * dss);
                    z1h[i < LC ? i : 0] = fma(cv.T.c, yb[i], cv.T.d * dss);
                }
                nd_total[i] = (live && cv.nd < (double)kNeverDrops) ? (int)cv.nd : (live ? kNeverDrops : 0);
            }
#pragma unroll
            for (int d = 1; d < SIG_WAVE; d <<= 1) {
                int other[VPT];
#pragma unroll
                for (int i = 0; i < VPT; ++i) other[i] = __shfl_xor(nd_total[i], d, SIG_WAVE);
#pragma unroll
                for (int i = 0; i < VPT; ++i) nd_total[i] = (other[i] > nd_total[i]) ? other[i] : nd_total[i];
            }
#pragma unroll
            for (int i = 0; i < VPT; ++i) nd_total[i] = __builtin_amdgcn_readfirstlane(nd_total[i]);
        }
        int drop_at[LC];
#pragma unroll
        for (int i = 0; i < LC; ++i) {
            drop_at[i] = (nd_total[i] > c) ? nd_total[i] - c : 0;
            if (drop_at[i] > 0) {
                const int v = (v0 + i < a.voices) ? v0 + i : vc;
                const double dss = fma(k2c[i], yb[i], -ya[i]) - yb[i];
                if constexpr (!CROWS) {
                    const double* t = sc + (int64_t)tk * a.voices + v;
                    z0h[i] = fma(t[0], yb[i], t[a.voices] * dss);
                    z1h[i] = fma(t[2 * (int64_t)a.voices], yb[i], t[3 * (int64_t)a.voices] * dss);
                }
            } else {
                z0h[i] = 0.0; z1h[i] = 0.0;
            }
        }
        int done = 0;
        auto single = [&]() {
            row(stage.slot, kTileStride, std::integral_constant<int, LC>{}, std::false_type{});
#pragma unroll
            for (int i = 0; i < VPT; ++i) { const double t = ya[i]; ya[i] = yb[i]; yb[i] = t; }
            ++done;
            stage.advance();
        };
        while (stage.staged != 0 && done < a.N) single();
        const int last_group_row = done + ((a.N - done) / R) * R;
        auto phase = [&](auto k_tag) {
            constexpr int K = decltype(k_tag)::value;
            constexpr int M = Variants::at(K);
            constexpr int lower = (K + 1 < Variants::count) ? Variants::at(K + 1) : 0;
            int until = 0;
#pragma unroll
            for (int i = lower; i < LC; ++i) until = (i < M && drop_at[i] > until) ? drop_at[i] : until;
            if (M == 0) until = a.N;
            until = (until < last_group_row) ? until : last_group_row;
            while (done < until) {
                group(std::integral_constant<int, M>{});
                done += R;
            }
        };
#define SIG_PHASE(K) if constexpr (K < Variants::count) phase(std::integral_constant<int, K>{});
        SIG_PHASE(0) SIG_PHASE(1) SIG_PHASE(2) SIG_PHASE(3) SIG_PHASE(4) SIG_PHASE(5) SIG_PHASE(6) SIG_PHASE(7) SIG_PHASE(8)
#undef SIG_PHASE
        if (done < a.N) {
            if (have) { folded.finish(pend, pend_row, R); have = false; }
#pragma unroll
            for (int i = 0; i < LC; ++i)
                if (drop_at[i] <= done) { z0h[i] = 0.0; z1h[i] = 0.0; }
            while (done < a.N) single();
        }
    }
    if (have) folded.finish(pend, pend_row, R);
    if (stage.staged) stage.now();
}

template <int VPT, int C, bool GROWS = false, bool CROWS = false>
__global__ __launch_bounds__(256) __attribute__((amdgpu_waves_per_eu(CROWS ? 1 : SteadyOcc<VPT>::waves, 8)))
void fused_steady_bus_kernel(FusedArgs a, BusArgs bus)
{
    __shared__ double lds[4][kPairs * kTileStride];
    constexpr bool kOscInLds = CROWS && VPT >= 8;
    __shared__ double osc_lds[kOscInLds ? 4 * 5 * VPT * SIG_WAVE : 1];
    const int lane = threadIdx.x & 63;
    const int wave = __builtin_amdgcn_readfirstlane(threadIdx.x >> 6);
    steady_bus_wave<VPT, C, GROWS, CROWS>(a, bus, lds[wave], lane, wave,
                                          kOscInLds ? osc_lds + (size_t)wave * 5 * VPT * SIG_WAVE : nullptr);
    if (bus.out) sig_bus::sum_tiles_in_workgroup<C>(bus.partials, a.voice_tiles, bus.rows, a.span, a.K, a.N, bus.out, bus.out_ld, lane, wave);
}

int64_t steady_consts_offset(int voices, int64_t rows, int bus_channels) {
    return (int64_t)((voices + SIG_WAVE - 1) / SIG_WAVE) * rows * bus_channels;
}


#ifndef SIG_FUSED_PART_B
}
sig_fused::Tuning& sig_fused::tuning() {
    static Tuning t = [] {
        auto env = [](const char* name, int dflt) { const char* e = getenv(name); return e ? atoi(e) : dflt; };
        Tuning u;
        u.vpt = env("SIG_FUSED_VPT", 0); u.span = env("SIG_FUSED_SPAN", 0);
        u.steady = env("SIG_FUSED_STEADY", -1); u.scan = env("SIG_FUSED_SCAN", -1);
        if (u.steady == 2) { u.steady = 1; u.tile_sum_kernel = 1; }
        if (u.steady == 3) { u.steady = 1; u.mix_f32 = 1; }
        return u;
    }();
    return t;
}
namespace {
#endif

constexpr int64_t kWavesWanted = 2048;

void pick_geometry(const FusedArgs& a, int max_vpt, int& vpt, int& span) {
    const int env_vpt = tuning().vpt, env_span = tuning().span;
    const int max_span = (a.N >= a.ctx) ? 8 : 1;
    auto waves = [&](int v, int s) { return (int64_t)((a.voices + SIG_WAVE * v - 1) / (SIG_WAVE * v)) * ((a.K + s - 1) / s); };
    vpt = max_vpt; span = max_span;
    while (span > 1 && waves(vpt, span) < kWavesWanted) span >>= 1;
    while (vpt > 1 && waves(vpt, 1) < kWavesWanted / 2) vpt >>= 1;
    if (env_vpt == 1 || env_vpt == 2 || env_vpt == 4) vpt = (env_vpt <= max_vpt) ? env_vpt : max_vpt;
    if (env_span >= 1) span = (env_span <= max_span) ? env_span : max_span;
}

template <int KIND, bool GAIN, int C, bool ROWS = false>
int launch_walk(FusedArgs a, BusArgs bus, int vpt, hipStream_t stream)
{
    a.voice_tiles = (a.voices + SIG_WAVE * vpt - 1) / (SIG_WAVE * vpt);
    const int64_t nwg = ((int64_t)a.voice_tiles * ((a.K + a.span - 1) / a.span) + 3) / 4;
    if (nwg > 0x7fffffffLL) return (int)hipErrorInvalidValue;
    if constexpr (C < 0) {
        fused_walk_kernel<KIND, 1, GAIN, C, ROWS><<<(unsigned)nwg, 256, 0, stream>>>(a, bus);
    } else {
        switch (vpt) {
            case 1: fused_walk_kernel<KIND, 1, GAIN, C, ROWS><<<(unsigned)nwg, 256, 0, stream>>>(a, bus); break;
            case 2: fused_walk_kernel<KIND, 2, GAIN, C, ROWS><<<(unsigned)nwg, 256, 0, stream>>>(a, bus); break;
            case 4: fused_walk_kernel<KIND, 4, GAIN, C, ROWS><<<(unsigned)nwg, 256, 0, stream>>>(a, bus); break;
            default: return (int)hipErrorInvalidValue;
        }
    }
    return sig_launch_status();
}

struct BusPlan { int vpt, span, steady; };
BusPlan plan_voice_bus(const FusedArgs& a, int kind);
template <bool GAIN, int C, bool GROWS, bool CROWS = false>
int launch_steady(FusedArgs& a, BusArgs& bus, int vpt, float* out, int64_t out_ld, hipStream_t stream);

template <int KIND, int C>
int launch_rows(FusedArgs a, BusArgs bus, float* out, int64_t out_ld, hipStream_t stream)
{
    if constexpr (KIND == SIG_OSC_SINE && C > 0) {
        const bool gain_only = a.gain && a.gain_rows > 1 && a.cutoff_rows == 1;
        if ((gain_only || a.cutoff_rows > 1) && !a.hertz_hist && !a.phase_hist && a.pair_op == 0) {
            BusPlan plan = plan_voice_bus(a, KIND);
            if (plan.steady) {
                if (plan.vpt > 8) plan.vpt = 8;
                if (!gain_only && tuning().vpt == 0) plan.vpt = (plan.vpt >= 8) ? 8 : (plan.vpt > 2 ? 2 : plan.vpt);
                a.span = plan.span;
                a.steady = 1;
                const int err = gain_only ? launch_steady<false, C, true>(a, bus, plan.vpt, out, out_ld, stream)
                                          : launch_steady<false, C, true, true>(a, bus, plan.vpt, out, out_ld, stream);
                if (err || bus.out) return err;
                const int tiles_s = (a.voices + SIG_WAVE * plan.vpt - 1) / (SIG_WAVE * plan.vpt);
                return sig_bus::launch_partials<C>(bus.partials, tiles_s, bus.rows, out, out_ld, stream);
            }
        }
    }
    auto ok = [&](int vpt) {
        return C > 0 || ((a.voices % vpt == 0) && (a.out_ld % vpt == 0) && (reinterpret_cast<uintptr_t>(a.out) % (vpt * 4) == 0));
    };
    int max_vpt = 4;
    while (max_vpt > 1 && !ok(max_vpt)) max_vpt >>= 1;
    int vpt;
    pick_geometry(a, max_vpt, vpt, a.span);
    const int tiles = (a.voices + SIG_WAVE * vpt - 1) / (SIG_WAVE * vpt);
    if (C > 0 && sig_bus::tiles_sum_in_workgroup(tiles) && tuning().tile_sum_kernel == 0) { bus.out = out; bus.out_ld = out_ld; }
    const int err = launch_walk<KIND, false, C, true>(a, bus, vpt, stream);
    if (err || C == 0 || bus.out) return err;
    return sig_bus::launch_partials<(C > 0 ? C : 1)>(bus.partials, tiles, bus.rows, out, out_ld, stream);
}

template <int C>
int dispatch_rows_kind(int kind, const FusedArgs& a, const BusArgs& bus, float* out, int64_t out_ld, hipStream_t s)
{
    switch (kind) {
#if SIG_FUSED_HERE_SINE
        case SIG_OSC_SINE: return launch_rows<SIG_OSC_SINE, C>(a, bus, out, out_ld, s);
#endif
#if SIG_FUSED_HERE_OTHERS
        case SIG_OSC_SQUARE: return launch_rows<SIG_OSC_SQUARE, C>(a, bus, out, out_ld, s);
        case SIG_OSC_SAWTOOTH: return launch_rows<SIG_OSC_SAWTOOTH, C>(a, bus, out, out_ld, s);
        case SIG_OSC_TRIANGLE: return launch_rows<SIG_OSC_TRIANGLE, C>(a, bus, out, out_ld, s);
#elif SIG_FUSED_SPLIT
        case SIG_OSC_SQUARE: case SIG_OSC_SAWTOOTH: case SIG_OSC_TRIANGLE: return part_b_rows(C, kind, a, bus, out, out_ld, s);
#endif
    }
    return (int)hipErrorInvalidValue;
}

BusPlan plan_voice_bus(const FusedArgs& a, int kind) {
    BusPlan p{4, 1, 0};
    pick_geometry(a, 4, p.vpt, p.span);
    if (kind == SIG_OSC_SINE && !a.force_walk && (a.N >= a.ctx || a.position >= a.ctx)) {
        p.steady = tuning().steady < 0 ? 1 : tuning().steady;
        if (p.steady) {
            const int env_vpt = tuning().vpt;
            auto waves = [&](int v, int s) { return (int64_t)((a.voices + SIG_WAVE * v - 1) / (SIG_WAVE * v)) * ((a.K + s - 1) / s); };
            if (env_vpt == 8 || (env_vpt == 0 && p.vpt == 4 && waves(8, p.span) >= kWavesWanted / 2)) p.vpt = 8;
            if (env_vpt == 16 || (SIG_STEADY_AUTO16 && env_vpt == 0 && p.vpt == 8 && a.voices >= SIG_WAVE * 16)) {
                int span = p.span;
                while (span > 1 && waves(16, span) < kWavesWanted / 2) span >>= 1;
                if (env_vpt == 16 || waves(16, span) >= kWavesWanted / 2) {
                    p.vpt = 16;
                    if (tuning().span == 0) p.span = span;
                }
            }
        }
    }
    return p;
}

template <bool GAIN, int C, bool GROWS, bool CROWS>
int launch_steady(FusedArgs& a, BusArgs& bus, int vpt, float* out, int64_t out_ld, hipStream_t stream)
{
    double* consts = a.consts_ext ? a.consts_ext : bus.partials + steady_consts_offset(a.voices, bus.rows, C);
    a.steady_consts = consts;
    if (!(a.consts_ext && a.consts_ready))
        steady_prep_kernel<GAIN><<<(a.voices + 255) / 256, 256, 0, stream>>>(a, consts);

    a.voice_tiles = (a.voices + SIG_WAVE * vpt - 1) / (SIG_WAVE * vpt);
    const int64_t nwg = ((int64_t)a.voice_tiles * ((a.K + a.span - 1) / a.span) + 3) / 4;
    if (nwg > 0x7fffffffLL) return (int)hipErrorInvalidValue;
    if (sig_bus::tiles_sum_in_workgroup(a.voice_tiles) && tuning().tile_sum_kernel == 0) { bus.out = out; bus.out_ld = out_ld; }
    switch (vpt) {
        case 1: fused_steady_bus_kernel<1, C, GROWS, CROWS><<<(unsigned)nwg, 256, 0, stream>>>(a, bus); break;
        case 2: fused_steady_bus_kernel<2, C, GROWS, CROWS><<<(unsigned)nwg, 256, 0, stream>>>(a, bus); break;
        case 8: fused_steady_bus_kernel<8, C, GROWS, CROWS><<<(unsigned)nwg, 256, 0, stream>>>(a, bus); break;
        case 16: if constexpr (!CROWS) { fused_steady_bus_kernel<16, C, GROWS><<<(unsigned)nwg, 256, 0, stream>>>(a, bus); break; }
        default: fused_steady_bus_kernel<4, C, GROWS, CROWS><<<(unsigned)nwg, 256, 0, stream>>>(a, bus); break;
    }
    return sig_launch_status();
}

template <int KIND, bool GAIN, int C>
int launch_voice_bus(FusedArgs a, BusArgs bus, float* out, int64_t out_ld, hipStream_t stream)
{
    const BusPlan plan = plan_voice_bus(a, KIND);
    const int vpt = plan.vpt;
    a.span = plan.span;
    a.steady = plan.steady;
    bool done = false;
    if constexpr (KIND == SIG_OSC_SINE) {
        if (a.steady) {
            const int e2 = launch_steady<GAIN, C, false>(a, bus, vpt, out, out_ld, stream);
            if (e2 || bus.out) return e2;
            done = true;
        }
    }
    if (!done) {
        const int tiles_w = (a.voices + SIG_WAVE * vpt - 1) / (SIG_WAVE * vpt);
        if (sig_bus::tiles_sum_in_workgroup(tiles_w) && tuning().tile_sum_kernel == 0) { bus.out = out; bus.out_ld = out_ld; }
        const int err = launch_walk<KIND, GAIN, C>(a, bus, vpt, stream);
        if (err || bus.out) return err;
    }
    const int tiles = (a.voices + SIG_WAVE * vpt - 1) / (SIG_WAVE * vpt);
    return sig_bus::launch_partials<C>(bus.partials, tiles, bus.rows, out, out_ld, stream);
}

template <int KIND, bool GAIN>
int dispatch_bus_channels(int C, const FusedArgs& a, const BusArgs& bus, float* out, int64_t out_ld, hipStream_t s)
{
    switch (C) {
#ifndef SIG_TUNE_SINE_ONLY
        case 1: return launch_voice_bus<KIND, GAIN, 1>(a, bus, out, out_ld, s);
        case 4: return launch_voice_bus<KIND, GAIN, 4>(a, bus, out, out_ld, s);
#endif
        case 2: return launch_voice_bus<KIND, GAIN, 2>(a, bus, out, out_ld, s);
    }
    return (int)hipErrorInvalidValue;
}

template <bool GAIN>
int dispatch_bus_kind(int kind, int C, const FusedArgs& a, const BusArgs& bus, float* out, int64_t out_ld, hipStream_t s)
{
    switch (kind) {
#if SIG_FUSED_HERE_SINE
        case SIG_OSC_SINE: return dispatch_bus_channels<SIG_OSC_SINE, GAIN>(C, a, bus, out, out_ld, s);
#endif
#if SIG_FUSED_HERE_OTHERS
        case SIG_OSC_SQUARE: return dispatch_bus_channels<SIG_OSC_SQUARE, GAIN>(C, a, bus, out, out_ld, s);
        case SIG_OSC_SAWTOOTH: return dispatch_bus_channels<SIG_OSC_SAWTOOTH, GAIN>(C, a, bus, out, out_ld, s);
        case SIG_OSC_TRIANGLE: return dispatch_bus_channels<SIG_OSC_TRIANGLE, GAIN>(C, a, bus, out, out_ld, s);
#elif SIG_FUSED_SPLIT
        case SIG_OSC_SQUARE: case SIG_OSC_SAWTOOTH: case SIG_OSC_TRIANGLE: return part_b_bus(GAIN ? 1 : 0, kind, C, a, bus, out, out_ld, s);
#endif
    }
    return (int)hipErrorInvalidValue;
}

constexpr int kScanMaxL = 8;


template <int KIND, bool GAIN>
__global__ __launch_bounds__(256) void fused_scan_kernel(FusedArgs a)
{
    const int lane = threadIdx.x & 63;
    const int64_t item = (int64_t)blockIdx.x * 4 + (threadIdx.x >> 6);
    const int v = (int)(item % a.voices);
    const int64_t b = item / a.voices;
    if (b >= a.K) return;
    const int64_t p_b = (a.pos_dev ? *a.pos_dev : a.position) + b * a.N;
    const int c = (int)((p_b < (int64_t)a.ctx) ? p_b : (int64_t)a.ctx);
    const int64_t n0 = p_b - c;
    const int total = c + a.N;
    const int L = (total + SIG_WAVE - 1) / SIG_WAVE;

    Biquad q;
    const bool ok = design_butter2(a.type, a.cutoff[(int64_t)v * a.cs], a.rate, q);
    if (!ok && a.status && lane == 0) atomicOr(a.status, SIG_STATUS_BAD_CUTOFF);
    const double hz = a.hertz[(int64_t)v * a.hs];
    const double ph = a.phase ? a.phase[(int64_t)v * a.ps] : 0.0;
    const double g = GAIN ? a.gain[(int64_t)v * a.gs] : 1.0;

    double yl[kScanMaxL];
    double z0 = 0.0, z1 = 0.0;
#pragma unroll
    for (int k = 0; k < kScanMaxL; ++k) {
        const int r = lane * L + k;
        const bool valid = (k < L) && (r < total);
        const double t = (double)(n0 + r) / a.rate * hz + ph;
        double x = (KIND == SIG_OSC_SINE) ? (double)sig_osc::osc_sine_f32(t) : sig_osc::osc_wave_fused<KIND>(t);
        x = valid ? x : 0.0;
        const double y = fma(q.b0, x, z0);
        const double nz0 = fma(q.b1, x, fma(-q.a1, y, z1));
        const double nz1 = fma(q.b2, x, -q.a2 * y);
        yl[k] = y;
        if (k < L) { z0 = nz0; z1 = nz1; }
    }

    const M2 A = {-q.a1, 1.0, -q.a2, 0.0};
    M2 M = A;
    for (int k = 1; k < L; ++k) M = m2_mul(A, M);
    double s0 = z0, s1 = z1;
#pragma unroll
    for (int d = 1; d < SIG_WAVE; d <<= 1) {
        const double p0 = __hiloint2double(__shfl_up(__double2hiint(s0), d, SIG_WAVE), __shfl_up(__double2loint(s0), d, SIG_WAVE));
        const double p1 = __hiloint2double(__shfl_up(__double2hiint(s1), d, SIG_WAVE), __shfl_up(__double2loint(s1), d, SIG_WAVE));
        if (lane >= d) {
            s0 += fma(M.a, p0, M.b * p1);
            s1 += fma(M.c, p0, M.d * p1);
        }
        M = m2_mul(M, M);
    }
    double t0 = __hiloint2double(__shfl_up(__double2hiint(s0), 1, SIG_WAVE), __shfl_up(__double2loint(s0), 1, SIG_WAVE));
    double t1 = __hiloint2double(__shfl_up(__double2hiint(s1), 1, SIG_WAVE), __shfl_up(__double2loint(s1), 1, SIG_WAVE));
    if (lane == 0) { t0 = 0.0; t1 = 0.0; }

    float* dst = a.out + (b * a.N - c) * a.out_ld + v;
#pragma unroll
    for (int k = 0; k < kScanMaxL; ++k) {
        const int r = lane * L + k;
        const double yh = t0;
        const double y = yl[k] + yh;
        const double u0 = fma(-q.a1, yh, t1);
        t1 = -q.a2 * yh;
        t0 = u0;
        if (k < L && r >= c && r < total) dst[(int64_t)r * a.out_ld] = (float)(GAIN ? y * g : y);
    }
}


constexpr int64_t kScanMaxChains = 16384;

template <int KIND, bool GAIN>
int launch_fused(FusedArgs a, hipStream_t stream)
{
    {
        const int scan_env = tuning().scan;
        const int64_t chains = (int64_t)a.voices * a.K;
        const bool fits = a.ctx + a.N <= kScanMaxL * SIG_WAVE;
        const bool want = scan_env >= 0 ? scan_env != 0 : chains <= kScanMaxChains;
        if (fits && want) {
            const int64_t nwg = (chains + 3) / 4;
            if (nwg > 0x7fffffffLL) return (int)hipErrorInvalidValue;
            fused_scan_kernel<KIND, GAIN><<<(unsigned)nwg, 256, 0, stream>>>(a);
            return sig_launch_status();
// ... 172 lines not shown
    }
    return (int)hipErrorInvalidValue;
}
}

extern "C" int sig_fused_osc_pair_biquad(int osc_kind, int osc2_kind, int pair_op, int filt_type, int32_t rate, int64_t position,
                                         int32_t block_frames, int32_t nblocks, int32_t context, int32_t voices,
                                         const double* hertz, int32_t hertz_stride, const double* phase, int32_t phase_stride,
                                         const double* hertz2, int32_t hertz2_stride, const double* phase2, int32_t phase2_stride,
                                         const double* mix, int32_t mix_stride,
                                         const double* cutoff, int32_t cutoff_stride, int32_t cutoff_rows,
                                         const double* gain, int32_t gain_stride, int32_t gain_rows,
                                         float* out, int64_t out_ld, int32_t* status, void* stream)
{
    SIG_CHECK_ARG(pair_op == 1 || pair_op == 2);
    return fused_chain_general(osc_kind, filt_type, rate, position, block_frames, nblocks, context, voices, hertz, hertz_stride, phase,
                               phase_stride, PairSource{pair_op, osc2_kind, hertz2, hertz2_stride, phase2, phase2_stride, mix, mix_stride},
                               cutoff, cutoff_stride, cutoff_rows, gain, gain_stride, gain_rows, out, out_ld, status, stream);
}

extern "C" int sig_fused_voice_pair_bus(int osc_kind, int osc2_kind, int pair_op, int filt_type, int32_t rate, int64_t position,
                                        int32_t block_frames, int32_t nblocks, int32_t context, int32_t voices,
                                        const double* hertz, int32_t hertz_stride, const double* phase, int32_t phase_stride,
                                        const double* hertz2, int32_t hertz2_stride, const double* phase2, int32_t phase2_stride,
                                        const double* mix, int32_t mix_stride,
                                        const double* cutoff, int32_t cutoff_stride, int32_t cutoff_rows,
                                        const double* gain, int32_t gain_stride, int32_t gain_rows,
                                        const double* bus_gains, int64_t bus_gains_ld, int32_t bus_channels,
                                        double* workspace, float* out, int64_t out_ld, int32_t* status, void* stream)
{
    SIG_CHECK_ARG(pair_op == 1 || pair_op == 2);
    return fused_bus_general(osc_kind, filt_type, rate, position, block_frames, nblocks, context, voices, hertz, hertz_stride, phase,
                             phase_stride, PairSource{pair_op, osc2_kind, hertz2, hertz2_stride, phase2, phase2_stride, mix, mix_stride},
                             cutoff, cutoff_stride, cutoff_rows, gain, gain_stride, gain_rows, bus_gains, bus_gains_ld, bus_channels,
                             workspace, out, out_ld, status, stream);
}

extern "C" int sig_fused_osc_biquad_rows(int osc_kind, int filt_type, int32_t rate, int64_t position,
                                         int32_t block_frames, int32_t nblocks, int32_t context, int32_t voices,
                                         const double* hertz, int32_t hertz_stride, const double* phase, int32_t phase_stride,
                                         const double* cutoff, int32_t cutoff_stride, int32_t cutoff_rows,
                                         const double* gain, int32_t gain_stride, int32_t gain_rows,
                                         float* out, int64_t out_ld, int32_t* status, void* stream)
{
    return fused_chain_general(osc_kind, filt_type, rate, position, block_frames, nblocks, context, voices, hertz, hertz_stride, phase,
                               phase_stride, PairSource{}, cutoff, cutoff_stride, cutoff_rows, gain, gain_stride, gain_rows, out, out_ld,
                               status, stream);
}

extern "C" int sig_fused_voice_bus_rows(int osc_kind, int filt_type, int32_t rate, int64_t position,
                                        int32_t block_frames, int32_t nblocks, int32_t context, int32_t voices,
                                        const double* hertz, int32_t hertz_stride, const double* phase, int32_t phase_stride,
                                        const double* cutoff, int32_t cutoff_stride, int32_t cutoff_rows,
                                        const double* gain, int32_t gain_stride, int32_t gain_rows,
                                        const double* bus_gains, int64_t bus_gains_ld, int32_t bus_channels,
                                        double* workspace, float* out, int64_t out_ld, int32_t* status, void* stream)
{
    return fused_bus_general(osc_kind, filt_type, rate, position, block_frames, nblocks, context, voices, hertz, hertz_stride, phase,
                             phase_stride, PairSource{}, cutoff, cutoff_stride, cutoff_rows, gain, gain_stride, gain_rows, bus_gains,
                             bus_gains_ld, bus_channels, workspace, out, out_ld, status, stream);
}

extern "C" int sig_fused_osc_biquad_fm(int osc_kind, int filt_type, int32_t rate, int64_t position,
                                       int32_t block_frames, int32_t nblocks, int32_t context, int32_t voices,
                                       const double* hertz, int32_t hertz_stride, int32_t hertz_rows, const double* hertz_hist,
                                       const double* phase, int32_t phase_stride, int32_t phase_rows, const double* phase_hist,
                                       const double* cutoff, int32_t cutoff_stride, int32_t cutoff_rows,
                                       const double* gain, int32_t gain_stride, int32_t gain_rows,
                                       float* out, int64_t out_ld, int32_t* status, void* stream)
{
    return fused_chain_general(osc_kind, filt_type, rate, position, block_frames, nblocks, context, voices, hertz, hertz_stride, phase,
                               phase_stride, PairSource{}, cutoff, cutoff_stride, cutoff_rows, gain, gain_stride, gain_rows, out, out_ld,
                               status, stream, FmSource{hertz_rows, phase_rows, hertz_hist, phase_hist});
}

extern "C" int sig_fused_voice_bus_fm(int osc_kind, int filt_type, int32_t rate, int64_t position,
                                      int32_t block_frames, int32_t nblocks, int32_t context, int32_t voices,
                                      const double* hertz, int32_t hertz_stride, int32_t hertz_rows, const double* hertz_hist,
                                      const double* phase, int32_t phase_stride, int32_t phase_rows, const double* phase_hist,
                                      const double* cutoff, int32_t cutoff_stride, int32_t cutoff_rows,
                                      const double* gain, int32_t gain_stride, int32_t gain_rows,
                                      const double* bus_gains, int64_t bus_gains_ld, int32_t bus_channels,
                                      double* workspace, float* out, int64_t out_ld, int32_t* status, void* stream)
{
    return fused_bus_general(osc_kind, filt_type, rate, position, block_frames, nblocks, context, voices, hertz, hertz_stride, phase,
                             phase_stride, PairSource{}, cutoff, cutoff_stride, cutoff_rows, gain, gain_stride, gain_rows, bus_gains,
                             bus_gains_ld, bus_channels, workspace, out, out_ld, status, stream,
                             FmSource{hertz_rows, phase_rows, hertz_hist, phase_hist});
}

extern "C" int sig_fused_osc_biquad_devpos(int osc_kind, int filt_type, int32_t rate, const int64_t* position_dev,
                                           int32_t block_frames, int32_t nblocks, int32_t context, int32_t voices,
                                           const double* hertz, int32_t hertz_stride, const double* phase, int32_t phase_stride,
                                           const double* cutoff, int32_t cutoff_stride,
                                           const double* gain, int32_t gain_stride,
                                           float* out, int64_t out_ld, int32_t* status, void* stream)
{
    SIG_CHECK_ARG(filt_type == SIG_FILT_LOWPASS || filt_type == SIG_FILT_HIGHPASS);
    SIG_CHECK_ARG(rate > 0 && position_dev && block_frames >= 0 && nblocks >= 0 && context >= 0 && voices >= 0);
    SIG_CHECK_ARG(hertz && cutoff && out && out_ld >= voices);
    SIG_CHECK_ARG((hertz_stride | 1) == 1 && (phase_stride | 1) == 1 && (cutoff_stride | 1) == 1 && (gain_stride | 1) == 1);
    if (block_frames == 0 || nblocks == 0 || voices == 0) return 0;
    FusedArgs a{filt_type, (double)rate, 0, block_frames, nblocks, context, voices,
                hertz, hertz_stride, phase, phase_stride, cutoff, cutoff_stride, gain, gain_stride,
                out, out_ld, 0, status, position_dev};
    hipStream_t s = static_cast<hipStream_t>(stream);
    return gain ? dispatch_kind<true>(osc_kind, a, s) : dispatch_kind<false>(osc_kind, a, s);
}

namespace {
__global__ void advance_kernel(int64_t* p, int64_t delta) { *p += delta; }
}

extern "C" int sig_advance_position(int64_t* position_dev, int64_t delta, void* stream)
{
    SIG_CHECK_ARG(position_dev != nullptr);
    advance_kernel<<<1, 1, 0, static_cast<hipStream_t>(stream)>>>(position_dev, delta);
    return sig_launch_status();
}

extern "C" int sig_fused_osc_biquad_mix(int osc_kind, int filt_type, int32_t rate, int64_t position,
                                        int32_t block_frames, int32_t nblocks, int32_t context, int32_t voices,
                                        const double* hertz, int32_t hertz_stride, const double* phase, int32_t phase_stride,
                                        const double* cutoff, int32_t cutoff_stride,
                                        const double* gain, int32_t gain_stride,
                                        const float* matrix, float* out, int64_t out_ld, int32_t* status, void* stream)
{
    SIG_CHECK_ARG(filt_type == SIG_FILT_LOWPASS || filt_type == SIG_FILT_HIGHPASS);
    SIG_CHECK_ARG(rate > 0 && position >= 0 && block_frames >= 0 && nblocks >= 0 && context >= 0 && voices >= 0);
    SIG_CHECK_ARG(hertz && cutoff && matrix && out && out_ld >= voices && voices % 64 == 0);
    SIG_CHECK_ARG((hertz_stride | 1) == 1 && (phase_stride | 1) == 1 && (cutoff_stride | 1) == 1 && (gain_stride | 1) == 1);
    if (block_frames == 0 || nblocks == 0 || voices == 0) return 0;
    FusedArgs a{filt_type, (double)rate, position, block_frames, nblocks, context, voices,
                hertz, hertz_stride, phase, phase_stride, cutoff, cutoff_stride, gain, gain_stride,
                out, out_ld, 0, status};
    a.mix = matrix;
    hipStream_t s = static_cast<hipStream_t>(stream);
    return gain ? dispatch_mix_kind<true>(osc_kind, a, s) : dispatch_mix_kind<false>(osc_kind, a, s);
}

extern "C" int sig_fused_geometry(int32_t voices, int32_t block_frames, int32_t nblocks, int32_t context,
                                  int32_t* voices_per_lane, int32_t* blocks_per_lane)
{
    SIG_CHECK_ARG(voices >= 0 && block_frames >= 0 && nblocks >= 0 && context >= 0 && voices_per_lane && blocks_per_lane);
    FusedArgs a{};
    a.N = block_frames; a.K = nblocks; a.ctx = context; a.voices = voices;
    int vpt = 1, span = 1;
    pick_geometry(a, 4, vpt, span);
    *voices_per_lane = vpt;
    *blocks_per_lane = span;
    return 0;
}

extern "C" int sig_fused_voice_bus_plan(int osc_kind, int64_t position, int32_t voices, int32_t block_frames, int32_t nblocks,
                                       int32_t context, int32_t* voices_per_lane, int32_t* blocks_per_lane,
                                       int32_t* closed_form)
{
    SIG_CHECK_ARG(voices >= 0 && block_frames >= 0 && nblocks >= 0 && context >= 0 && position >= 0);
    SIG_CHECK_ARG(voices_per_lane && blocks_per_lane && closed_form);
    FusedArgs a{};
    a.position = position; a.N = block_frames; a.K = nblocks; a.ctx = context; a.voices = voices;
    const BusPlan p = plan_voice_bus(a, osc_kind);
    *voices_per_lane = p.vpt;
    *blocks_per_lane = p.span;
    *closed_form = p.steady;
    return 0;
}

extern "C" int sig_fused_set_tuning(int32_t voices_per_lane, int32_t blocks_per_lane, int32_t closed_form, int32_t scan)
{
    SIG_CHECK_ARG(voices_per_lane >= 0 && blocks_per_lane >= 0 && closed_form >= -1 && closed_form <= 3 && scan >= -1);
    Tuning& t = tuning();
    t.vpt = voices_per_lane; t.span = blocks_per_lane; t.scan = scan;
    t.steady = (closed_form == 2 || closed_form == 3) ? 1 : closed_form;
    t.tile_sum_kernel = (closed_form == 2) ? 1 : 0;
    t.mix_f32 = (closed_form == 3) ? 1 : 0;
    return 0;
}

extern "C" int64_t sig_fused_voice_bus_workspace(int32_t voices, int64_t rows, int32_t bus_channels)
{
    return (steady_consts_offset(voices, rows, bus_channels) + (int64_t)kSteadyConsts * voices) * (int64_t)sizeof(double);
}

namespace {
int fused_voice_bus_impl(int osc_kind, int filt_type, int32_t rate, int64_t position,
                         int32_t block_frames, int32_t nblocks, int32_t context, int32_t voices,
                         const double* hertz, int32_t hertz_stride, const double* phase, int32_t phase_stride,
                         const double* cutoff, int32_t cutoff_stride, const double* gain, int32_t gain_stride,
                         const double* bus_gains, int64_t bus_gains_ld, int32_t bus_channels,
                         double* workspace, float* out, int64_t out_ld, int32_t* status, void* stream,
                         double* consts, int32_t consts_ready, int force_walk = 0)
{
    SIG_CHECK_ARG(filt_type == SIG_FILT_LOWPASS || filt_type == SIG_FILT_HIGHPASS);
    SIG_CHECK_ARG(rate > 0 && position >= 0 && block_frames >= 0 && nblocks >= 0 && context >= 0 && voices >= 0);
    SIG_CHECK_ARG(hertz && cutoff && out && workspace && out_ld >= bus_channels);
    SIG_CHECK_ARG((hertz_stride | 1) == 1 && (phase_stride | 1) == 1 && (cutoff_stride | 1) == 1 && (gain_stride | 1) == 1);
    SIG_CHECK_ARG(bus_gains ? bus_gains_ld >= voices : bus_channels == 1);
    if (block_frames == 0 || nblocks == 0 || voices == 0) return 0;
    FusedArgs a{filt_type, (double)rate, position, block_frames, nblocks, context, voices,
                hertz, hertz_stride, phase, phase_stride, cutoff, cutoff_stride, gain, gain_stride,
                nullptr, 0, 0, status};
    a.consts_ext = consts;
    a.consts_ready = consts_ready;
    a.force_walk = force_walk;
    BusArgs bus{bus_gains, bus_gains_ld, workspace, (int64_t)block_frames * nblocks};
    hipStream_t s = static_cast<hipStream_t>(stream);
    return gain ? dispatch_bus_kind<true>(osc_kind, bus_channels, a, bus, out, out_ld, s)
                : dispatch_bus_kind<false>(osc_kind, bus_channels, a, bus, out, out_ld, s);
}
}

extern "C" int sig_fused_voice_bus(int osc_kind, int filt_type, int32_t rate, int64_t position,
                                   int32_t block_frames, int32_t nblocks, int32_t context, int32_t voices,
                                   const double* hertz, int32_t hertz_stride, const double* phase, int32_t phase_stride,
                                   const double* cutoff, int32_t cutoff_stride,
                                   const double* gain, int32_t gain_stride,
                                   const double* bus_gains, int64_t bus_gains_ld, int32_t bus_channels,
                                   double* workspace, float* out, int64_t out_ld, int32_t* status, void* stream)
{
    return fused_voice_bus_impl(osc_kind, filt_type, rate, position, block_frames, nblocks, context, voices, hertz, hertz_stride,
                                phase, phase_stride, cutoff, cutoff_stride, gain, gain_stride, bus_gains, bus_gains_ld,
                                bus_channels, workspace, out, out_ld, status, stream, nullptr, 0);
}

extern "C" int sig_fused_voice_bus_walk(int osc_kind, int filt_type, int32_t rate, int64_t position,
                                        int32_t block_frames, int32_t nblocks, int32_t context, int32_t voices,
                                        const double* hertz, int32_t hertz_stride, const double* phase, int32_t phase_stride,
                                        const double* cutoff, int32_t cutoff_stride,
                                        const double* gain, int32_t gain_stride,
                                        const double* bus_gains, int64_t bus_gains_ld, int32_t bus_channels,
                                        double* workspace, float* out, int64_t out_ld, int32_t* status, void* stream)
{
    return fused_voice_bus_impl(osc_kind, filt_type, rate, position, block_frames, nblocks, context, voices, hertz, hertz_stride,
                                phase, phase_stride, cutoff, cutoff_stride, gain, gain_stride, bus_gains, bus_gains_ld,
                                bus_channels, workspace, out, out_ld, status, stream, nullptr, 0, 1);
}

extern "C" int64_t sig_fused_voice_consts_size(int32_t voices)
{
    return (int64_t)kSteadyConsts * voices * (int64_t)sizeof(double);
}

extern "C" int sig_fused_voice_bus_prepared(int osc_kind, int filt_type, int32_t rate, int64_t position,
                                            int32_t block_frames, int32_t nblocks, int32_t context, int32_t voices,
                                            const double* hertz, int32_t hertz_stride, const double* phase, int32_t phase_stride,
                                            const double* cutoff, int32_t cutoff_stride,
                                            const double* gain, int32_t gain_stride,
                                            const double* bus_gains, int64_t bus_gains_ld, int32_t bus_channels,
                                            double* workspace, float* out, int64_t out_ld, int32_t* status, void* stream,
                                            double* consts, int32_t consts_ready)
{
    SIG_CHECK_ARG(consts != nullptr);
    return fused_voice_bus_impl(osc_kind, filt_type, rate, position, block_frames, nblocks, context, voices, hertz, hertz_stride,
                                phase, phase_stride, cutoff, cutoff_stride, gain, gain_stride, bus_gains, bus_gains_ld,
                                bus_channels, workspace, out, out_ld, status, stream, consts, consts_ready);
}

extern "C" int sig_fused_voice_bus_bound(const sig_fused_voice_bus_call* c, int64_t position, float* out, int32_t consts_ready,
                                         int32_t walk, void* stream)
{
    SIG_CHECK_ARG(c != nullptr && (walk || c->consts != nullptr));
    return fused_voice_bus_impl(c->osc_kind, c->filt_type, c->rate, position, c->block_frames, c->nblocks, c->context, c->voices,
                                c->hertz, c->hertz_stride, c->phase, c->phase_stride, c->cutoff, c->cutoff_stride, c->gain, c->gain_stride,
                                c->bus_gains, c->bus_gains_ld, c->bus_channels, c->workspace, out, c->out_ld, c->status, stream,
                                walk ? nullptr : c->consts, walk ? 0 : consts_ready, walk ? 1 : 0);
}
#endif
```

### signals_amd/csrc/sig_bus_tile.h

```cpp
#pragma once
#include "sig_common.h"

namespace sig_bus {

constexpr int kPairs = 16;
constexpr int kTileStride = 65;
constexpr int kTileDoubles = kPairs * kTileStride;

__device__ __forceinline__ double sum16(const double (&pv)[16]) {
    const double a0 = pv[0] + pv[1], a1 = pv[2] + pv[3], a2 = pv[4] + pv[5], a3 = pv[6] + pv[7];
    const double a4 = pv[8] + pv[9], a5 = pv[10] + pv[11], a6 = pv[12] + pv[13], a7 = pv[14] + pv[15];
    const double b0 = a0 + a1, b1 = a2 + a3, b2 = a4 + a5, b3 = a6 + a7;
    return (b0 + b1) + (b2 + b3);
}

template <int C>
struct Tile {
    static constexpr int R = kPairs / C;
    double* tile; const double* col; double* dstp;
    int lane;

    __device__ __forceinline__ Tile(double* tile_, int lane_, double* dstp_)
        : tile(tile_), col(tile_ + (lane_ & (kPairs - 1)) * kTileStride + (lane_ >> 4) * 16), dstp(dstp_), lane(lane_) {}

    __device__ __forceinline__ void put(int k, const double (&acc)[C]) {
#pragma unroll
        for (int ch = 0; ch < C; ++ch) tile[(k * C + ch) * kTileStride + lane] = acc[ch];
    }
    template <bool AGENT = false>
    __device__ __forceinline__ void flush(int64_t out_row0, int k_lo, int k_hi) {
        double pv[16];
#pragma unroll
        for (int k = 0; k < 16; ++k) pv[k] = col[k];
        const double s = sig_sum_rows_f64(sum16(pv));
        const int k = lane / C;
        if (lane < kPairs && k >= k_lo && k < k_hi) {
            if (AGENT) __hip_atomic_store(dstp + (out_row0 + k) * C + lane % C, s, __ATOMIC_RELAXED, __HIP_MEMORY_SCOPE_AGENT);
            else dstp[(out_row0 + k) * C + lane % C] = s;
        }
    }
};

template <int C>
struct PipelinedTile {
    static constexpr int R = kPairs / C;
    double* tile; const double* col; double* slot; double* dstp;
    int lane, staged;
    int64_t first;

    __device__ __forceinline__ PipelinedTile(double* tile_, int lane_, double* dstp_, int64_t first_row)
        : tile(tile_), col(tile_ + (lane_ & (kPairs - 1)) * kTileStride + (lane_ >> 4) * 16), slot(tile_ + lane_),
          dstp(dstp_), lane(lane_), staged(0), first(first_row) {}

    __device__ __forceinline__ void issue(double (&pv)[16]) const {
#pragma unroll
        for (int k = 0; k < 16; ++k) pv[k] = col[k];
    }
    __device__ __forceinline__ void finish(const double (&pv)[16], int64_t row0, int nrows) const {
        const double s = sig_sum_rows_f64(sum16(pv));
        if (lane < nrows * C) dstp[row0 * C + lane] = s;
    }
    __device__ __forceinline__ void now() {
        double pv[16];
        issue(pv);
        finish(pv, first, staged);
        first += staged;
        staged = 0;
        slot = tile + lane;
    }
    __device__ __forceinline__ double* at(int k) const { return tile + k * C * kTileStride + lane; }
    __device__ __forceinline__ void advance() {
        slot += C * kTileStride;
        if (++staged == R) now();
    }
};

constexpr int kFoldStride = 17;

template <int C>
struct FoldedGroup {
    double* put; const double* get; double* dstp; int lane;
    __device__ __forceinline__ FoldedGroup(double* tile, int lane_, double* dstp_)
        : put(tile + ((((lane_ >> 4) & 1) << 1) | (lane_ >> 5)) * kFoldStride + (lane_ & 15)),
          get(tile + (lane_ & 15) * kFoldStride + 4 * (lane_ >> 4)), dstp(dstp_), lane(lane_) {}
    __device__ __forceinline__ void fold4(int q, double t0, double t1, double t2, double t3) const {
        put[4 * q * kFoldStride] = sig_fold16(sig_fold32(t0, t1), sig_fold32(t2, t3));
    }
    __device__ __forceinline__ void issue(double (&pv)[4]) const {
#pragma unroll
        for (int t = 0; t < 4; ++t) pv[t] = get[t];
    }
    __device__ __forceinline__ void finish(const double (&pv)[4], int64_t row0, int nrows) const {
        const double s = sig_sum_rows_f64((pv[0] + pv[1]) + (pv[2] + pv[3]));
        if (lane < nrows * C) dstp[row0 * C + lane] = s;
    }
};

constexpr bool tiles_sum_in_workgroup(int tiles) { return tiles == 1 || tiles == 2 || tiles == 4; }

template <int C>
__device__ __forceinline__ void sum_tiles_in_workgroup(const double* partials, int tiles, int64_t rows, int span, int K, int N,
                                                       float* out, int64_t out_ld, int lane, int wave)
{
    asm volatile("s_waitcnt vmcnt(0)" ::: "memory");
    __syncthreads();
    const int64_t item = (int64_t)blockIdx.x * 4 + wave;
    const int t = (int)(item % tiles);
    const int64_t b_first = (item / tiles) * span;
    if (b_first >= K) return;
    const int nb = (int)((K - b_first < (int64_t)span) ? K - b_first : (int64_t)span);
    const int64_t n = (int64_t)nb * N * C, first = b_first * N * C, per = (n + tiles - 1) / tiles;
    const int64_t lo = first + t * per, hi = (first + n < lo + per) ? first + n : lo + per;
    constexpr int U = 8;
    int64_t i = lo + lane;
    for (; i + (U - 1) * SIG_WAVE < hi; i += U * SIG_WAVE) {
        double s[U];
#pragma unroll
        for (int u = 0; u < U; ++u) s[u] = 0.0;
        for (int k = 0; k < tiles; ++k) {
            const double* src = partials + (int64_t)k * rows * C + i;
#pragma unroll
            for (int u = 0; u < U; ++u) s[u] += src[u * SIG_WAVE];
        }
#pragma unroll
        for (int u = 0; u < U; ++u) {
            const int64_t j = i + u * SIG_WAVE;
            out[(j / C) * out_ld + (j % C)] = (float)s[u];
        }
    }
    for (; i < hi; i += SIG_WAVE) {
        double s = 0.0;
        for (int k = 0; k < tiles; ++k) s += partials[(int64_t)k * rows * C + i];
        out[(i / C) * out_ld + (i % C)] = (float)s;
    }
}

template <int C>
static __global__ __launch_bounds__(256) void partials_kernel(const double* __restrict__ partials, int tiles, int64_t rows,
                                                               float* __restrict__ out, int64_t out_ld)
{
    const int64_t n = rows * C;
    for (int64_t i = (int64_t)blockIdx.x * blockDim.x + threadIdx.x; i < n; i += (int64_t)gridDim.x * blockDim.x) {
        double s = 0.0;
        for (int t = 0; t < tiles; ++t) s += partials[(int64_t)t * n + i];
        out[(i / C) * out_ld + (i % C)] = (float)s;
    }
}

template <int C>
static int launch_partials(const double* partials, int tiles, int64_t rows, float* out, int64_t out_ld, hipStream_t stream)
{
    const int64_t n = rows * C;
    int64_t g = (n + 255) / 256;
    if (g > 4096) g = 4096;
    partials_kernel<C><<<(unsigned)g, 256, 0, stream>>>(partials, tiles, rows, out, out_ld);
    return sig_launch_status();
}

}
```

### signals_amd/engine.py

```python
from __future__ import annotations

import os
import typing

import torch

from signals_amd import _native, runtime
from signals_amd.chain import (
    AUDIO_DTYPE,
    CTRL_DTYPE,
    Emitter,
    Receiver,
    as_control,
    broadcast_shape,
    graph_clock,
    port,
)
from signals_amd.chain import ext, files, fixed, fx, noise, osc, shape

CONTEXT = 100
SCAN_MAX_CHAINS = 16384
SCAN_MAX_ROWS = 512


# ... 1050 lines not shown
    def impure_outputs(self):
        return self._impure.items()


def _deal_over_tiles(order: torch.Tensor, voices_per_lane: int) -> torch.Tensor:
    tile = 64 * voices_per_lane
    tiles = order.shape[0] // tile
    perm = order.clone()
    if tiles:
        q = torch.arange(tiles * tile, device=order.device)
        group, lane = q // 64, q % 64
        perm[((group % tiles) * 64 + lane) * voices_per_lane + group // tiles] = order[q]
    return perm


class _VoiceChain:

    def __init__(self, batch: _Batch, src, filt, gain_node, bus_node, channels: int, pre_gain=None, pair=None):
        self.batch, self.src, self.filt, self.gain_node, self.bus_node = batch, src, filt, gain_node, bus_node
        self.pre_gain = pre_gain
        self.pair = pair
        self.pair_rows = None
        self.channels = channels
        self.gain_ports = [g.right for g in (pre_gain, gain_node) if g is not None]
        self.ports = [src.hertz, src.phase, filt.cutoff] + self.gain_ports
        self.involved = [n for n in (src, filt, gain_node, bus_node, pre_gain, *(pair or ())) if n is not None]
        self.kind, self.btype = src.kind(), str(filt.type())
        self.fm = not (_ctl_const(src.hertz) and _ctl_const(src.phase))
        self.hist_rows = (None, None)
        self.modulated = self.fm or any(not _ctl_const(p) for p in [filt.cutoff] + self.gain_ports)
        self.general = self.modulated or pair is not None
        source = self.kind if pair is None else f'{type(pair[0]).__name__}({self.kind},{pair[1].kind()})'
        self.tag = (f'{source},{self.btype}{",gain" if self.gain_ports else ""}{",per-block" if self.modulated else ""}'
                    f'{",fm" if self.fm else ""}')
        if pair is not None:
            self.ports += [pair[1].hertz, pair[1].phase] + ([pair[0].mix] if isinstance(pair[0], fx.Mix) else [])

    @classmethod
    def match_and_launch(cls, batch: _Batch, node: Emitter, channels: int, hist: int) -> torch.Tensor | None:
        bus_node, mix_node, top = None, None, node
        if isinstance(node, ext.SumBus):
            if not batch.owner.fuse_bus or hist != 0 or node.channels not in (1, 2, 4):
                return None
            bus_node, top = node, node.input.sig
            if top is None or not top.get_state().enabled or len(top.outputs_with_ports) != 1:
                return None
            channels = node.input.channels
        elif isinstance(node, ext.MixMatrix):
            if hist != 0 or channels % 64:
                return None
            mix_node, top = node, node.input.sig
            if top is None or not top.get_state().enabled or len(top.outputs_with_ports) != 1:
                return None
        gain_node, filt = None, top
        if isinstance(top, fx.Gain):
            gain_node, filt = top, top.left.sig
            if not isinstance(filt, fx.SingleCritFilter) or len(filt.outputs_with_ports) != 1:
                return None
        if not isinstance(filt, fx.SingleCritFilter) or not filt.get_state().enabled:
            return None
        src, pre_gain = filt.input.sig, None
        if (isinstance(src, fx.Gain) and src.get_state().enabled and _ctl_const(src.right) and isinstance(src.left.sig, osc.Osc)
                and (src, channels) not in batch._memo):
            pre_gain, src = src, src.left.sig
        pair = None
        if (pre_gain is None and isinstance(src, (fx.Mix, fx.RingMod)) and src.get_state().enabled and not _modulated(src)
                and len(src.outputs_with_ports) == 1 and (src, channels) not in batch._memo):
            left, right = src.left.sig, src.right.sig
            if (isinstance(left, osc.Osc) and isinstance(right, osc.Osc) and left is not right and right.get_state().enabled
                    and len(right.outputs_with_ports) == 1 and _ctl_const(right.hertz) and _ctl_const(right.phase)):
                pair, src = (src, right), left
        if not isinstance(src, osc.Osc) or not src.get_state().enabled or len(src.outputs_with_ports) != 1:
            return None
        fm = not (_ctl_const(src.hertz) and _ctl_const(src.phase))
        if fm and (pair is not None or batch.N < CONTEXT):
            return None
        chain = cls(batch, src, filt, gain_node, bus_node, channels, pre_gain, pair)
        controls = chain.resolve()
        if controls is None or not chain.widths_ok(controls):
            return None
        if mix_node is not None:
            return chain.launch_mix(mix_node, controls)
        return chain.launch_bus(node, controls) if bus_node is not None else chain.launch_chain(node, controls, hist)

    def resolve(self):
        if not all(n.get_state().enabled for n in self.involved):
            return None
        try:
            if self.pair is not None:
                op, second = self.pair
                self.pair_rows = (self.batch._control_const(second.hertz, 'hertz'), self.batch._control_const(second.phase, 'phase'),
                                  self.batch._control_const(op.mix, 'mix') if isinstance(op, fx.Mix) else None)
            if self.modulated:
                b, o = self.batch, self.batch.owner
                ports = self.ports[:2] + [self.filt.cutoff] + self.gain_ports
                q = -1
                if self.fm:
                    contiguous = o._stream_end == b.pos and bool(o._prev_block_frames) and o._prev_block_frames >= min(CONTEXT, b.pos)
                    q = b.pos - (o._prev_block_frames if contiguous else min(CONTEXT, b.pos))
                got = b._control_many(ports, q, channels=self.channels)
                vals, fronts = (got, None) if q < 0 else got
                vals = [as_control(t) for t in vals]
                rows, gains = vals[:3], vals[3:]
                if self.fm:
                    self.hist_rows = tuple(None if _ctl_const(p) else as_control(f) for p, f in zip(self.ports[:2], fronts[:2]))
                if len(gains) == 2:
                    gains = [(gains[0] * gains[1]).contiguous()]
                return rows + (gains or [None])
            rows = [self.batch._control_const(p, p.name) for p in self.ports[:2]]
            rows.append(self.batch._control_const(self.filt.cutoff, 'cutoff'))
            gains = [self.batch._control_const(p, p.name) for p in self.gain_ports]
        except NotBatchable:
            return None
        if len(gains) == 2:
            held = self.batch.owner._gain_products.get((id(gains[0]), id(gains[1])))
            if held is None or held[0] is not gains[0] or held[1] is not gains[1]:
                self.batch.owner._gain_products.clear()
                held = self.batch.owner._gain_products[(id(gains[0]), id(gains[1]))] = (gains[0], gains[1], (gains[0] * gains[1]).contiguous())
            gains = [held[2]]
        return rows + (gains or [None])

    def widths_ok(self, controls) -> bool:
        hertz, phase, cutoff, gain = controls
        v = self.channels
        source = [hertz, phase] + [t for t in (self.pair_rows or ()) if t is not None]
        return (max(t.shape[1] for t in source) == v and cutoff.shape[1] == v
                and all(t.shape[1] in (1, v) for t in source) and (gain is None or gain.shape[1] in (1, v)))

    def pair_arg(self):
        if self.pair is None:
            return None
        return (type(self.pair[0]).__name__, self.pair[1].kind(), *self.pair_rows)

    def cycles_per_frame_bound(self) -> tuple[float, float]:
        import numpy as np
        out = []
        for p in (self.src.hertz, self.src.phase):
            src = p.sig
            if src is None or not src._state.enabled:
                out.append(0.0)
            else:
                value = np.abs(np.asarray(src._state.value, dtype=np.float64))
                out.append(float(value.max()) if value.size and np.isfinite(value).all() else float('inf'))
        return out[0] / self.batch.rate, out[1]

    def ordered_by_cutoff(self, ctl, pan, voices_per_lane: int):
        index = self.cutoff_order(ctl, voices_per_lane)
        if index is None:
            return ctl, pan
        v = self.channels
        pick = lambda t: t if t is None or t.shape[1] != v else t.index_select(1, index).contiguous()
        return [pick(t) for t in ctl], pick(pan)

    def cutoff_order(self, ctl, voices_per_lane: int):
        import numpy as np
        v, src = self.channels, self.filt.cutoff.sig
        if ctl[2].shape[1] != v or not isinstance(src, fixed.Fixed):
            return None
        cut = np.asarray(src._state.value, dtype=np.float64).reshape(-1)
        if cut.size != v or not np.isfinite(cut).all():
            return None
        return _deal_over_tiles(torch.from_numpy(np.argsort(cut, kind='stable')), voices_per_lane).to(runtime.device())

    def live_key(self, bus_node=None):
        for n in self.involved:
            if not n._state.enabled:
                return None
        key = []
        for p in self.ports:
            src = p.sig
            if src is None or not src._state.enabled:
                key.append(None)
            elif type(src) is fixed.Fixed:
                key.append(src.resident())
            else:
                return None
        if bus_node is not None:
            key.append(bus_node.resident_gains())
        return key

    def _same_shapes(self, now, then) -> bool:
        return now is not None and all(a.shape == b.shape for a, b in zip(now[:3], then[:3]))

    def launch_chain(self, node: Emitter, controls, hist: int) -> torch.Tensor:
        b, o, dev = self.batch, self.batch.owner, runtime.device()
        N, K, rate, v = b.N, b.K, b.rate, self.channels
        rows = N * K
        status = o._status_word(self.filt)
        name = f'fused_osc_biquad[{self.tag}]'

        def run(position, ctl, out):
            if self.general:
                return o._launch(name, lambda: _native.fused_rows(self.kind, self.btype, rate, position, N, K, CONTEXT, v,
                                                                  ctl[0], ctl[1], ctl[2], ctl[3], out, status=status,
                                                                  pair=self.pair_arg(), hertz_hist=self.hist_rows[0],
                                                                  phase_hist=self.hist_rows[1]),
                                 units=rows * v)
            return o._launch(name, lambda: _native.fused_osc_biquad(self.kind, self.btype, rate, position, N, K, CONTEXT,
                                                                    ctl[0], ctl[1], ctl[2], ctl[3], out, status=status),
                             units=rows * v)
        if hist:
            result = torch.empty((hist + rows, v), dtype=AUDIO_DTYPE, device=dev)
            run(b.pos, controls, result[hist:])
            b._own_history(node, v, hist, result)
            return result

        def replay(position: int) -> torch.Tensor:
            ctl = self.resolve()
            if not self._same_shapes(ctl, controls):
                o._replay = None
                return o.render(position, N, K)
            return run(position, ctl, torch.empty((rows, v), dtype=AUDIO_DTYPE, device=dev))
        if node is o.node and not self.modulated:
            o._remember_replay(N, K, replay)
        return run(b.pos, controls, torch.empty((rows, v), dtype=AUDIO_DTYPE, device=dev))

    def launch_mix(self, mix_node, controls) -> torch.Tensor:
        b, o = self.batch, self.batch.owner
        N, K, v = b.N, b.K, self.channels
        if self.general:
            return None
        out = torch.empty((N * K, v), dtype=AUDIO_DTYPE, device=runtime.device())
        matrix, status = mix_node.resident_matrix(), o._status_word(self.filt)
        return o._launch(f'fused_osc_biquad_mix[{self.tag}]',
                         lambda: _native.fused_osc_biquad_mix(self.kind, self.btype, b.rate, b.pos, N, K, CONTEXT,
                                                              controls[0], controls[1], controls[2], controls[3], matrix, out,
                                                              status=status),
                         units=N * K * v)

    def launch_bus(self, node: Emitter, controls) -> torch.Tensor:
        b, o, dev = self.batch, self.batch.owner, runtime.device()
        N, K, rate, v = b.N, b.K, b.rate, self.channels
        rows, bus_c = N * K, self.bus_node.channels
        pan = self.bus_node.resident_gains()
        if pan is not None and pan.shape[1] != v:
            return None
        status = o._status_word(self.filt)
        o._bus_workspace(v, rows, bus_c)
        if self.general:
            if bus_c not in (1, 2):
                return None
            swept = controls[2].shape[0] > 1
            if (self.kind == 'Sine' and self.pair is None and not self.fm and controls[2].shape[1] == v
                    and (swept or (controls[3] is not None and controls[3].shape[0] > 1 and controls[3].shape[1] == v))):
                held = o._tremolo_order
                key = (id(controls[0]), id(controls[1]), id(controls[2]) if not swept else None, id(pan), K, swept)
                if held is None or held[0] != key:
                    plan = _native.fused_voice_bus_plan('Sine', b.pos, v, N, K, CONTEXT)
                    vpl = min(plan['voices_per_lane'], 8)
                    if swept and vpl < 8:
                        vpl = min(vpl, 2)
                    if not plan['closed_form']:
                        index = None
                    elif not swept:
                        index = self.cutoff_order(controls, vpl)
                    else:
                        index = _deal_over_tiles(torch.argsort(controls[2][0], stable=True), vpl)
                    pick = lambda t: t if t is None or index is None or t.shape[1] != v else t.index_select(1, index).contiguous()
                    held = o._tremolo_order = (key, (controls[0], controls[1], controls[2], pan), index,
                                               [pick(controls[0]), pick(controls[1]), None if swept else pick(controls[2])], pick(pan))
                if held[2] is not None:
                    pick = lambda t: t if t is None or t.shape[1] != v else t.index_select(1, held[2])
                    cut = pick(controls[2]) if swept else held[3][2]
                    gain_rows = controls[3]
                    if gain_rows is not None and gain_rows.shape[1] == v:
                        gain_rows = pick(gain_rows)
                    controls = [held[3][0], held[3][1], cut, gain_rows]
                    pan = held[4]
            out = torch.empty((rows, bus_c), dtype=AUDIO_DTYPE, device=dev)
            return o._launch(f'fused_voice_bus[{self.tag}]',
                             lambda: _native.fused_rows(self.kind, self.btype, rate, b.pos, N, K, CONTEXT, v, controls[0], controls[1],
                                                        controls[2], controls[3], out, bus_gains=pan, bus=True,
                                                        workspace=o._workspace, status=status, pair=self.pair_arg(),
                                                        hertz_hist=self.hist_rows[0], phase_hist=self.hist_rows[1]),
                             units=rows * v)
        small = v * K <= o.scan_max_chains and CONTEXT + N <= SCAN_MAX_ROWS
        chain_name, bus_name = f'fused_osc_biquad[{self.tag}]', f'fused_voice_bus[{self.tag}]'
        one_launch = small and K == 1 and self.kind == 'Sine' and o.latency_kernel
        if one_launch and (o._latency_ws is None or o._latency_ws[0] != (v, N, bus_c)):
            o._latency_ws = ((v, N, bus_c), _native.latency_voice_bus_workspace(v, N, bus_c, dev))

        def run(position, ctl, pan_now, out):
            if one_launch:
                return o._launch(f'latency_voice_bus[{self.tag}]',
                                 lambda: _native.latency_voice_bus(self.btype, rate, position, N, CONTEXT, v, ctl[0], ctl[1],
                                                                   ctl[2], ctl[3], pan_now, out, o._latency_ws[1],
                                                                   status=status), units=rows * v)
            if small:
                voices_buf = torch.empty((rows, v), dtype=AUDIO_DTYPE, device=dev)
                o._launch(chain_name, lambda: _native.fused_osc_biquad(self.kind, self.btype, rate, position, N, K, CONTEXT,
                                                                       ctl[0], ctl[1], ctl[2], ctl[3], voices_buf,
                                                                       status=status), units=rows * v)
                return o._launch('sum_bus', lambda: _native.sum_bus(voices_buf, pan_now, out), units=rows * v)
            key = (tuple(id(t) for t in ctl), id(pan_now), self.btype, rate, v, min(CONTEXT, position))
            held = o._steady_consts
            ready = held is not None and held[0] == key
            if not ready:
                size = _native.lib().sig_fused_voice_consts_size(v) // 8
                buf = held[2] if held is not None and held[2].numel() >= size else torch.empty(size, dtype=CTRL_DTYPE, device=dev)
                plan = _native.fused_voice_bus_plan(self.kind, position, v, N, K, CONTEXT)
                o._steady_consts = held = (key, (tuple(ctl), pan_now), buf, self.cycles_per_frame_bound(),
                                           self.ordered_by_cutoff(ctl, pan_now, plan['voices_per_lane']))
            ctl, pan_now = held[4]
            per_frame, ph_max = held[3]
            walk = self.kind == 'Sine' and ph_max + (position + rows) * per_frame >= _native.SINE_FAST_MAX_CYCLES
            if o.timer is None or o.timer.region:
                call = held[5] if len(held) > 5 else None
                if call is None or call.shape != (rows, bus_c) or call._keep[5] is not o._workspace:
                    call = _native.FusedVoiceBusCall(self.kind, self.btype, rate, N, K, CONTEXT, v, ctl[0], ctl[1], ctl[2], ctl[3], pan_now,
                                                     bus_c, o._workspace, status, held[2])
                    o._steady_consts = held = (*held[:5], call)
                if o.timer is not None:
                    return o.timer.launch(bus_name, lambda: call(position, out, ready, walk), units=rows * v)
                return call(position, out, ready, walk)
            return o._launch(bus_name, lambda: _native.fused_voice_bus(self.kind, self.btype, rate, position, N, K, CONTEXT, v,
                                                                       ctl[0], ctl[1], ctl[2], ctl[3], pan_now, out,
                                                                       workspace=o._workspace, status=status,
                                                                       consts=held[2], consts_ready=ready, walk=walk),
                             units=rows * v)

        def captured(position, ctl, pan_now):
            keys = tuple(t.data_ptr() if t is not None else 0 for t in (*ctl, pan_now))
            cap = o._captured
            if cap is None or cap.keys != keys:
                def record(pos_t: torch.Tensor) -> torch.Tensor:
                    bus_out = torch.empty((rows, bus_c), dtype=AUDIO_DTYPE, device=dev)
                    if one_launch:
                        return _native.latency_voice_bus(self.btype, rate, pos_t, N, CONTEXT, v, ctl[0], ctl[1], ctl[2], ctl[3],
                                                         pan_now, bus_out, o._latency_ws[1], status=status)
                    vbuf = torch.empty((rows, v), dtype=AUDIO_DTYPE, device=dev)
                    _native.fused_osc_biquad(self.kind, self.btype, rate, pos_t, N, K, CONTEXT,
                                             ctl[0], ctl[1], ctl[2], ctl[3], vbuf, status=status)
                    return _native.sum_bus(vbuf, pan_now, bus_out)
                try:
                    cap = o._captured = _CapturedLaunches(record, N * K, position, keys, self_advancing=one_launch)
                except RuntimeError:
                    o.graph_replay, o._captured = False, None
                    return None
            return cap.run(position)

        bound = [None]

        RING = 4

        def pipelined(position: int):
            key = self.live_key(self.bus_node)
            held, pipe = o._steady_consts, o._pipe
            if key is None or held is None or len(held) < 5 or held[0][-1] != CONTEXT or position < CONTEXT:
                return None
            if pipe is None or pipe['held'] is not held or len(pipe['key']) != len(key) or not all(a is b for a, b in zip(key, pipe['key'])) \
                    or pipe['shape'] != (rows, bus_c):
                held_ctl, held_pan = held[1]
                if len(key) != len(held_ctl) + 1 or key[-1] is not held_pan or \
                        not all(k is None or k is t for k, t in zip(key, held_ctl)):
                    return None
                torch.cuda.synchronize()
                ctl_o, pan_o = held[4]
                ws_size = _native.lib().sig_fused_voice_bus_workspace(v, rows, bus_c) // 8
                streams = [torch.cuda.Stream() for _ in range(o.pipeline)]
                work = [torch.empty(ws_size, dtype=CTRL_DTYPE, device=dev) for _ in streams]
                pipe = o._pipe = {
                    'held': held, 'key': key, 'shape': (rows, bus_c), 'i': 0, 'streams': streams, 'work': work,
                    'handles': [s_.cuda_stream for s_ in streams],
                    'events': [torch.cuda.Event() for _ in streams],
                    'calls': [_native.FusedVoiceBusCall(self.kind, self.btype, rate, N, K, CONTEXT, v, ctl_o[0], ctl_o[1], ctl_o[2], ctl_o[3],
                                                        pan_o, bus_c, w, status, held[2]) for w in work],
                    'outs': [[torch.empty((rows, bus_c), dtype=AUDIO_DTYPE, device=dev) for _ in range(RING)] for _ in streams],
                    'slot': [0] * len(streams)}
                torch.cuda.synchronize()
            per_frame, ph_max = held[3]
            if self.kind == 'Sine' and ph_max + (position + rows) * per_frame >= _native.SINE_FAST_MAX_CYCLES:
                return None
            i = pipe['i']
            pipe['i'] = (i + 1) % len(pipe['streams'])
            slot = pipe['slot'][i]
            pipe['slot'][i] = (slot + 1) % RING
            out = pipe['outs'][i][slot]
            call, handle = pipe['calls'][i], pipe['handles'][i]
            if o.timer is not None:
                o.timer.launch(bus_name, lambda: call(position, out, True, False, stream=handle), units=rows * v)
            else:
                call(position, out, True, False, stream=handle)
            pipe['events'][i].record(pipe['streams'][i])
            raw = _native.current_stream_handle(dev.index)
            cur = pipe.get('current')
            if cur is None or cur[0] != raw:
                cur = pipe['current'] = (raw, torch.cuda.current_stream())
            cur[1].wait_event(pipe['events'][i])
            return out

        def replay(position: int) -> torch.Tensor:
            if o.pipeline > 1 and not small and (o.timer is None or o.timer.region):
                done = pipelined(position)
                if done is not None:
                    return done
            if one_launch and o.timer is None:
                key, held = self.live_key(self.bus_node), bound[0]
                if key is not None and held is not None and len(key) == len(held[0]) and all(a is b for a, b in zip(key, held[0])):
                    return held[1](position, torch.empty((rows, bus_c), dtype=AUDIO_DTYPE, device=dev))
            ctl, pan_now = self.resolve(), self.bus_node.resident_gains()
            if not self._same_shapes(ctl, controls) or (pan_now is None) != (pan is None):
                o._replay = None
                return o.render(position, N, K)
            if small and o.graph_replay and not one_launch:
                out = captured(position, ctl, pan_now)
                if out is not None:
                    return out
            if one_launch and o.timer is None:
                key = self.live_key(self.bus_node)
                if key is not None and (pan_now is None or pan_now.shape[1] == v) and self.widths_ok(ctl):
                    bound[0] = (key, _native.LatencyVoiceBusCall(self.btype, rate, N, CONTEXT, v, ctl[0], ctl[1], ctl[2], ctl[3],
                                                                 pan_now, bus_c, o._latency_ws[1], status))
            return run(position, ctl, pan_now, torch.empty((rows, bus_c), dtype=AUDIO_DTYPE, device=dev))
        if node is o.node:
            o._remember_replay(N, K, replay)
        return run(b.pos, controls, pan, torch.empty((rows, bus_c), dtype=AUDIO_DTYPE, device=dev))


class _NoProgram(Exception):
    """this graph is not one voice program"""


class _ProgramRows:

    def __init__(self, srcs: tuple, K: int, lead: int, small: bool, channels: int | None = None, status=None):
        self.srcs, self.K, self.lead, self.small = srcs, K, lead, small
        more = dict(channels=channels, status=status)
        if not small:
            self.main = _ControlProgram(srcs, K, lead=lead, **more)
            self.full = self.main.full
            self.front = [_ControlProgram(srcs, 1, into={i: t[j:j + 1] for i, t in self.full.items()}, **more) for j in range(lead - 1)]
        else:
            probe = _ControlProgram(srcs, K, lead=K, **more)
            self.main, self.full = probe, probe.full
            if probe.windowed:
                raise NotBatchable('a filter in a control path with blocks of <= 100 frames (the next block is served from the '
                                   'after-window cache)')
            self.virtual = _ControlProgram(srcs, K, into={i: t[:K] for i, t in self.full.items()}, **more)
            self.first = _ControlProgram(srcs, 1, into={i: t[K:K + 1] for i, t in self.full.items()}, **more)

    def current(self) -> bool:
        return self.main.current()

    def tensors(self) -> list:
        return [self.full.get(i, r if r is not None else as_control(src.resident()))
                for i, (src, r) in enumerate(zip(self.srcs, self.main.results))]


class _VoiceProgram:

    KERNEL_NODES = (osc.Osc, fx.SingleCritFilter, fx.DoubleCritFilter, fx.Gain, fx.Amp, fx.Mix, fx.RingMod, ext.ADSR, noise.White,
                    ext.PMOsc)

    def __init__(self, batch: '_Batch', top: Emitter, voices: int):
        self.batch, self.top, self.voices = batch, top, voices
        self.code: list = []
        self.oscs: list = []
        self.params: list = []
        self.filters: list = []
        self.bands: list = []
        self.controls: list = []
        self.adsr = None
        self.seeds: list = []
        self.temps_used, self.temps_free, self.n_temps = set(), [], 0
        self.saved: dict = {}
        self.depth_of: dict = {}
        self.uses: dict = {}
        self.kernel_nodes = 0
        self._count(top)
        for n, uses in self.uses.items():
            if n is not top and len(n.outputs_with_ports) != uses:
                raise _NoProgram(f'{n.cls_name()} has a reader outside the graph')
        self.depth = self._emit(top, 0)
        if len(self.code) > _native.VP_MAX_INS:
            raise _NoProgram('program too long')
        if self.bands and any(op == 'OscPM' for op, *_ in self.code):
            raise _NoProgram('a band filter and a phase-modulation oscillator: no interpreter variant has both')

    def _count(self, n):
        if n is None or not n.get_state().enabled:
            if isinstance(n, ext.Tap):
                self._count(n.input.sig)
            return
        if isinstance(n, ext.Tap):
            return self._count(n.input.sig)
        self.uses[n] = self.uses.get(n, 0) + 1
        if self.uses[n] > 1:
            return
        if isinstance(n, self.KERNEL_NODES):
            self.kernel_nodes += 1
        elif not isinstance(n, fixed.Fixed):
            raise _NoProgram(f'no voice-program instruction for {n.cls_name()}')
        for port in _audio_ports(n):
            self._count(port.sig)

    def _control(self, port, below: int, optional: bool = False):
        src = port.sig
        if src is None or not src.get_state().enabled:
            if optional:
                return None
            self.controls.append((None, Emitter.empty_result(), below))
        else:
            self.controls.append((port, None, below))
        return len(self.controls) - 1

    def _param(self, index: int) -> int:
        if len(self.params) >= _native.VP_MAX_PARAMS:
            raise _NoProgram('more parameter registers than the machine has')
        self.params.append(index)
        return len(self.params) - 1

    def _temp(self) -> int:
        if self.temps_free:
            t = self.temps_free.pop()
        else:
            t = self.n_temps
            self.n_temps += 1
            if self.n_temps > _native.VP_MAX_TEMPS:
                raise _NoProgram('more temporaries than the machine has')
        return t

    def _zero(self, below: int) -> int:
        self.controls.append((None, Emitter.empty_result(), below))
        self.code.append(('Const', 0, self._param(len(self.controls) - 1), 0, 0))
        return 0

    def _osc_slot(self, n, below: int) -> int:
        if len(self.oscs) >= _native.VP_MAX_OSCS:
            raise _NoProgram('more oscillators than the machine has slots')
        self.oscs.append((self._control(n.hertz, below), self._control(n.phase, below, optional=True)))
        return len(self.oscs) - 1

    def _emit(self, n, below: int) -> int:
        if isinstance(n, ext.Tap):
            return self._emit(n.input.sig, below)
# ... 199 lines not shown
```

Measured before the change: 2.579 million Msamples/s.

## Vouch filter-transient decay on host to enable 16-voice steady kernel with direct output

Adds a host-side bound on how many rows each biquad's transient needs to decay, computed from the fixed hertz and cutoff values. When every slot beyond the first few in each 16-voice group has decayed within the context, a flag lets the planner choose the 16-voices-per-lane closed-form steady kernel, which keeps only a reduced set of live transient slots. It also adds a DIRECT variant that writes f32 output straight from the tile fold when there is a single voice tile, skipping the partials buffer and the separate in-workgroup tile sum. The per-row accumulation is restructured into chunks of 8 voices to limit register pressure. The decay bound is an analytic estimate, so if it is wrong, dropped transients become numeric error.

Result: no change. 2.569 million Msamples/s (-0.4%).

```diff
diff --git a/include/signals_amd.h b/include/signals_amd.h
--- a/include/signals_amd.h
+++ b/include/signals_amd.h
@@ -255,6 +255,10 @@
                        int32_t* voices_per_lane, int32_t* blocks_per_lane);
 int sig_fused_voice_bus_plan(int osc_kind, int64_t position, int32_t voices, int32_t block_frames, int32_t nblocks,
                              int32_t context, int32_t* voices_per_lane, int32_t* blocks_per_lane, int32_t* closed_form);
+int sig_fused_voice_bus_plan_for(int osc_kind, int64_t position, int32_t voices, int32_t block_frames, int32_t nblocks,
+                                 int32_t context, int32_t slots_decayed, int32_t* voices_per_lane, int32_t* blocks_per_lane,
+                                 int32_t* closed_form);
+int sig_fused_steady_live_slots(int32_t voices_per_lane);
 int sig_fused_set_tuning(int32_t voices_per_lane, int32_t blocks_per_lane, int32_t closed_form, int32_t scan);
 int sig_fused_voice_bus(int osc_kind, int filt_type, int32_t rate, int64_t position,
                         int32_t block_frames, int32_t nblocks, int32_t context, int32_t voices,
diff --git a/signals_amd/_native.py b/signals_amd/_native.py
--- a/signals_amd/_native.py
+++ b/signals_amd/_native.py
@@ -115,6 +115,8 @@
         'sig_fused_voice_bus_workspace': [i32, i64, i32],
         'sig_fused_voice_consts_size': [i32],
         'sig_fused_voice_bus_plan': [cint, i64, i32, i32, i32, i32, p32, p32, p32],
+        'sig_fused_voice_bus_plan_for': [cint, i64, i32, i32, i32, i32, i32, p32, p32, p32],
+        'sig_fused_steady_live_slots': [i32],
         'sig_fused_geometry': [i32, i32, i32, i32, p32, p32],
         'sig_fused_set_tuning': [i32, i32, i32, i32],
         'sig_fused_cascade_bus': [cint, cint, cint, i32, i64, i64, i32, i32, i32, i32] + [dp, i32] * 5 + env + bus + out,
@@ -544,9 +546,9 @@
         self._block_ref = ctypes.byref(self._block)
         self._bound = lib().sig_fused_voice_bus_bound
 
-    def __call__(self, position: int, out: torch.Tensor, consts_ready: bool, walk: bool = False, stream: int | None = None) -> torch.Tensor:
+    def __call__(self, position: int, out: torch.Tensor, consts_ready: int, walk: bool = False, stream: int | None = None) -> torch.Tensor:
         s = _stream(out) if stream is None else stream
-        err = self._bound(self._block_ref, position, out.data_ptr(), 1 if consts_ready else 0, 1 if walk else 0, s)
+        err = self._bound(self._block_ref, position, out.data_ptr(), int(consts_ready), 1 if walk else 0, s)
         if err:
             raise NativeError(f'sig_fused_voice_bus failed: hipError_t {err}')
         return out
@@ -705,13 +707,42 @@
            'sig_control_program_attached')
 
 
-def fused_voice_bus_plan(kind: str, position: int, voices: int, block_frames: int, nblocks: int, context: int) -> dict:
+def fused_voice_bus_plan(kind: str, position: int, voices: int, block_frames: int, nblocks: int, context: int,
+                         slots_decayed: bool = True) -> dict:
     vpt, span, closed = ctypes.c_int32(), ctypes.c_int32(), ctypes.c_int32()
-    _check(lib().sig_fused_voice_bus_plan(OSC_KINDS[kind], position, voices, block_frames, nblocks, context,
-                                          ctypes.byref(vpt), ctypes.byref(span), ctypes.byref(closed)),
-           'sig_fused_voice_bus_plan')
+    _check(lib().sig_fused_voice_bus_plan_for(OSC_KINDS[kind], position, voices, block_frames, nblocks, context,
+                                              1 if slots_decayed else 0, ctypes.byref(vpt), ctypes.byref(span), ctypes.byref(closed)),
+           'sig_fused_voice_bus_plan_for')
     kernel = f'fused_steady_bus_kernel<{vpt.value}, C>' if closed.value else f'fused_walk_kernel<{kind}, {vpt.value}, gain, C>'
     return {'voices_per_lane': vpt.value, 'blocks_per_lane': span.value, 'closed_form': bool(closed.value), 'kernel': kernel}
+
+
+def steady_decay_rows(btype: str, rate: float, hertz, cutoff, tol: float = 1e-9):
+    import numpy as np
+    hz, cut = np.asarray(hertz, dtype=np.float64).reshape(-1), np.asarray(cutoff, dtype=np.float64).reshape(-1)
+    with np.errstate(all='ignore'):
+        k = np.tan(np.pi * (cut / (rate / 2)) / 2); k2 = k * k; nrm = 1 / (1 + np.sqrt(2) * k + k2)
+        b0 = (k2 if btype == 'lp' else 1.0) * nrm
+        a1, a2 = 2 * (k2 - 1) * nrm, (1 - np.sqrt(2) * k + k2) * nrm
+        s2 = 2.0 if btype == 'lp' else -2.0
+        d = hz / rate; z = np.exp(-2j * np.pi * (d - np.rint(d)))
+        H = (1 + s2 * z + z * z) / (1 + a1 * z + a2 * z * z)
+        P = H - 1; Q = P / z - s2 + a1 * H
+        d2 = a2 - 0.25 * a1 * a1; f2 = 1 + 0.25 * a1 * a1 + d2
+        kappa = (f2 + np.sqrt(np.maximum(f2 * f2 - 4 * d2, 0))) / (2 * np.sqrt(d2))
+        amp = b0 * kappa * np.sqrt(np.abs(P) ** 2 + np.abs(Q) ** 2)
+        rows = np.where(amp > tol, np.ceil(np.log(tol / amp) / (0.5 * np.log(a2))) + 1, 0.0)
+        ok = (cut > 0) & (cut < rate / 2) & (d2 > 0) & (a2 > 0) & (a2 < 1) & np.isfinite(rows)
+    return np.where(ok, rows, np.inf)
+
+
+def steady_slots_decayed(decay_rows, context: int, voices_per_lane: int = 16, margin: int = 2) -> bool:
+    import numpy as np
+    nd = np.asarray(decay_rows, dtype=np.float64).reshape(-1)
+    if nd.size == 0 or nd.size % voices_per_lane:
+        return False
+    live = lib().sig_fused_steady_live_slots(voices_per_lane)
+    return bool((nd.reshape(-1, voices_per_lane)[:, live:] + margin <= context).all())
 
 
 def set_fused_tuning(voices_per_lane: int = 0, blocks_per_lane: int = 0, closed_form: int = -1, scan: int = -1) -> None:
@@ -758,7 +789,7 @@
         entry, name = lib().sig_fused_voice_bus_walk, 'sig_fused_voice_bus_walk'
     elif consts is not None:
         entry, name = lib().sig_fused_voice_bus_prepared, 'sig_fused_voice_bus_prepared'
-        tail = (_consts(consts, voices), 1 if consts_ready else 0)
+        tail = (_consts(consts, voices), int(consts_ready))
     _check(entry(OSC_KINDS[kind], FILT_TYPES[btype], rate, position, block_frames, nblocks, context, voices, *ptrs,
                  *_bus_gains(bus_gains, bus, voices), bus, workspace.data_ptr(), out.data_ptr(), out.stride(0), _ptr(status),
                  _stream(out), *tail), name)
diff --git a/signals_amd/csrc/fused_voice.hip b/signals_amd/csrc/fused_voice.hip
--- a/signals_amd/csrc/fused_voice.hip
+++ b/signals_amd/csrc/fused_voice.hip
@@ -412,14 +412,14 @@
     put(SC_T0 + 0, c.T0.a); put(SC_T0 + 1, c.T0.b); put(SC_T0 + 2, c.T0.c); put(SC_T0 + 3, c.T0.d);
 }
 
-template <int VPT, int C>
+template <int VPT, int C, bool DIRECT = false>
 __device__ __forceinline__ void steady_fallback_span(const FusedArgs& a, const BusArgs& bus, double* tile, int lane, int vt,
                                                   int64_t b_first, int nb, int v0)
 {
     const int vc = (v0 < a.voices) ? v0 : 0;
     const double* sc = a.steady_consts;
     const double s2 = (a.type == SIG_FILT_LOWPASS) ? 2.0 : -2.0;
-    sig_bus::PipelinedTile<C> stage(tile, lane, bus.partials + (int64_t)vt * bus.rows * C, b_first * a.N);
+    sig_bus::PipelinedTile<C, DIRECT> stage(tile, lane, bus.partials + (int64_t)vt * bus.rows * C, b_first * a.N, bus.out, bus.out_ld);
     for (int i = 0; i < VPT; ++i)
         if (v0 + i < a.voices && a.status && sc[(int64_t)SC_NA1 * a.voices + v0 + i] != sc[(int64_t)SC_NA1 * a.voices + v0 + i])
             atomicOr(a.status, SIG_STATUS_BAD_CUTOFF);
@@ -469,11 +469,15 @@
 }
 
 
+#ifndef SIG_STEADY_LIVE16
+#define SIG_STEADY_LIVE16 5
+#endif
+static_assert(SIG_STEADY_LIVE16 > 4 && SIG_STEADY_LIVE16 <= 8, "the 16-per-lane variant list is {LIVE16, 4, 3, 2, 1, 0}");
 template <int VPT> struct SteadyVariants {
-    static constexpr int count = (VPT >= 8) ? 7 : (VPT == 4) ? 4 : (VPT == 2) ? 3 : 2;
+    static constexpr int count = (VPT == 16) ? 6 : (VPT == 8) ? 7 : (VPT == 4) ? 4 : (VPT == 2) ? 3 : 2;
     static constexpr int at(int k) {
-        constexpr int v8[7] = {8, 6, 4, 3, 2, 1, 0}, v4[4] = {4, 2, 1, 0}, v2[3] = {2, 1, 0}, v1[2] = {1, 0};
-        return (VPT >= 8) ? v8[k] : (VPT == 4) ? v4[k] : (VPT == 2) ? v2[k] : v1[k];
+        constexpr int v16[6] = {SIG_STEADY_LIVE16, 4, 3, 2, 1, 0}, v8[7] = {8, 6, 4, 3, 2, 1, 0}, v4[4] = {4, 2, 1, 0}, v2[3] = {2, 1, 0}, v1[2] = {1, 0};
+        return (VPT == 16) ? v16[k] : (VPT == 8) ? v8[k] : (VPT == 4) ? v4[k] : (VPT == 2) ? v2[k] : v1[k];
     }
 };
 
@@ -488,7 +492,7 @@
 #endif
 template <int VPT> struct SteadyOcc { static constexpr int waves = (VPT == 16) ? SIG_STEADY_OCC16 : (VPT == 8) ? SIG_STEADY_OCC8 : 2; };
 
-template <int VPT, int C, bool GROWS, bool CROWS = false>
+template <int VPT, int C, bool GROWS, bool CROWS = false, bool DIRECT = false>
 __device__ __forceinline__ void steady_bus_wave(const FusedArgs& a, const BusArgs& bus, double* tile, int lane, int wave, double* osc_store = nullptr)
 {
     constexpr bool OSC_LDS = CROWS && VPT >= 8;
@@ -504,7 +508,7 @@
     const int vc = (v0 < a.voices) ? v0 : 0;
     const int64_t p0 = a.position + b_first * a.N;
     if (!steady_wave(a, v0, VPT, p0, nb)) {
-        steady_fallback_span<VPT, C>(a, bus, tile, lane, vt, b_first, nb, v0);
+        steady_fallback_span<VPT, C, DIRECT>(a, bus, tile, lane, vt, b_first, nb, v0);
         return;
     }
     const double* sc = a.steady_consts;
@@ -548,7 +552,7 @@
     for (int i = 0; i < VPT; ++i) nd_total[i] = __builtin_amdgcn_readfirstlane(nd_total[i]);
 
     double* dstp = bus.partials + (int64_t)vt * bus.rows * C;
-    sig_bus::PipelinedTile<C> stage(tile, lane, dstp, b_first * a.N);
+    sig_bus::PipelinedTile<C, DIRECT> stage(tile, lane, dstp, b_first * a.N, bus.out, bus.out_ld);
 
     if constexpr (LC < VPT) {
         const int c_min = (b_first == 0 && a.position < (int64_t)a.ctx) ? (int)a.position : a.ctx;
@@ -556,7 +560,7 @@
 #pragma unroll
         for (int i = LC; i < VPT; ++i) capped &= nd_total[i] <= c_min;
         if (!capped) {
-            steady_fallback_span<VPT, C>(a, bus, tile, lane, vt, b_first, nb, v0);
+            steady_fallback_span<VPT, C, DIRECT>(a, bus, tile, lane, vt, b_first, nb, v0);
             return;
         }
     }
@@ -602,38 +606,42 @@
             sums[ch * sums_stride] = acc;
         }
     };
-    sig_bus::FoldedGroup<C> folded(tile, lane, dstp);
+    sig_bus::FoldedGroup<C, DIRECT> folded(tile, lane, dstp, bus.out, bus.out_ld);
     double pend[4];
     int64_t pend_row = 0;
     bool have = false;
     auto rows2 = [&](double* sums, auto m_tag) {
         constexpr int M = decltype(m_tag)::value;
-        double y0[VPT], y1[VPT];
-#pragma unroll
-        for (int i = 0; i < VPT; ++i) {
-            y0[i] = yb[i];
-            ya[i] = fma(k2c[i], yb[i], -ya[i]);
-            y1[i] = ya[i];
-            yb[i] = fma(k2c[i], ya[i], -yb[i]);
-            if (i < M) {
-                const int j = i < LC ? i : 0;
-                const double h0 = z0h[j];
-                y0[i] += h0;
-                const double h1 = fma(na1[j], h0, z1h[j]);
-                y1[i] += h1;
-                z0h[j] = fma(na1[j], h1, na2[j] * h0);
-                z1h[j] = na2[j] * h1;
-            }
-        }
+        constexpr int H = (VPT > 8) ? 8 : VPT;
         double acc0[C], acc1[C];
 #pragma unroll
         for (int ch = 0; ch < C; ++ch) { acc0[ch] = 0.0; acc1[ch] = 0.0; }
 #pragma unroll
-        for (int i = 0; i < VPT; ++i) {
-#pragma unroll
-            for (int ch = 0; ch < C; ++ch) {
-                acc0[ch] = fma(wt[ch][i], y0[i], acc0[ch]);
-                acc1[ch] = fma(wt[ch][i], y1[i], acc1[ch]);
+        for (int i0 = 0; i0 < VPT; i0 += H) {
+            double y0[H], y1[H];
+#pragma unroll
+            for (int i = i0; i < i0 + H; ++i) {
+                y0[i - i0] = yb[i];
+                ya[i] = fma(k2c[i], yb[i], -ya[i]);
+                y1[i - i0] = ya[i];
+                yb[i] = fma(k2c[i], ya[i], -yb[i]);
+                if (i < M) {
+                    const int j = i < LC ? i : 0;
+                    const double h0 = z0h[j];
+                    y0[i - i0] += h0;
+                    const double h1 = fma(na1[j], h0, z1h[j]);
+                    y1[i - i0] += h1;
+                    z0h[j] = fma(na1[j], h1, na2[j] * h0);
+                    z1h[j] = na2[j] * h1;
+                }
+            }
+#pragma unroll
+            for (int i = i0; i < i0 + H; ++i) {
+#pragma unroll
+                for (int ch = 0; ch < C; ++ch) {
+                    acc0[ch] = fma(wt[ch][i], y0[i - i0], acc0[ch]);
+                    acc1[ch] = fma(wt[ch][i], y1[i - i0], acc1[ch]);
+                }
             }
         }
 #pragma unroll
@@ -774,7 +782,7 @@
     if (stage.staged) stage.now();
 }
 
-template <int VPT, int C, bool GROWS = false, bool CROWS = false>
+template <int VPT, int C, bool GROWS = false, bool CROWS = false, bool DIRECT = false>
 __global__ __launch_bounds__(256) __attribute__((amdgpu_waves_per_eu(CROWS ? 1 : SteadyOcc<VPT>::waves, 8)))
 void fused_steady_bus_kernel(FusedArgs a, BusArgs bus)
 {
@@ -783,9 +791,11 @@
     __shared__ double osc_lds[kOscInLds ? 4 * 5 * VPT * SIG_WAVE : 1];
     const int lane = threadIdx.x & 63;
     const int wave = __builtin_amdgcn_readfirstlane(threadIdx.x >> 6);
-    steady_bus_wave<VPT, C, GROWS, CROWS>(a, bus, lds[wave], lane, wave,
+    steady_bus_wave<VPT, C, GROWS, CROWS, DIRECT>(a, bus, lds[wave], lane, wave,
                                           kOscInLds ? osc_lds + (size_t)wave * 5 * VPT * SIG_WAVE : nullptr);
-    if (bus.out) sig_bus::sum_tiles_in_workgroup<C>(bus.partials, a.voice_tiles, bus.rows, a.span, a.K, a.N, bus.out, bus.out_ld, lane, wave);
+    if constexpr (!DIRECT) {
+        if (bus.out) sig_bus::sum_tiles_in_workgroup<C>(bus.partials, a.voice_tiles, bus.rows, a.span, a.K, a.N, bus.out, bus.out_ld, lane, wave);
+    }
 }
 
 int64_t steady_consts_offset(int voices, int64_t rows, int bus_channels) {
@@ -908,9 +918,11 @@
             const int env_vpt = tuning().vpt;
             auto waves = [&](int v, int s) { return (int64_t)((a.voices + SIG_WAVE * v - 1) / (SIG_WAVE * v)) * ((a.K + s - 1) / s); };
             if (env_vpt == 8 || (env_vpt == 0 && p.vpt == 4 && waves(8, p.span) >= kWavesWanted / 2)) p.vpt = 8;
-            if (env_vpt == 16 || (SIG_STEADY_AUTO16 && env_vpt == 0 && p.vpt == 8 && a.voices >= SIG_WAVE * 16)) {
+            const bool auto16 = SIG_STEADY_AUTO16 && env_vpt == 0 && p.vpt == 8 && a.voices == SIG_WAVE * 16 && (a.consts_ready & 2) &&
+                                a.position >= (int64_t)a.ctx && a.cutoff_rows == 1 && a.gain_rows == 1;
+            if (env_vpt == 16 || auto16) {
                 int span = p.span;
-                while (span > 1 && waves(16, span) < kWavesWanted / 2) span >>= 1;
+                while (span > (auto16 ? 2 : 1) && waves(16, span) < kWavesWanted / 2) span >>= 1;
                 if (env_vpt == 16 || waves(16, span) >= kWavesWanted / 2) {
                     p.vpt = 16;
                     if (tuning().span == 0) p.span = span;
@@ -926,13 +938,20 @@
 {
     double* consts = a.consts_ext ? a.consts_ext : bus.partials + steady_consts_offset(a.voices, bus.rows, C);
     a.steady_consts = consts;
-    if (!(a.consts_ext && a.consts_ready))
+    if (!(a.consts_ext && (a.consts_ready & 1)))
         steady_prep_kernel<GAIN><<<(a.voices + 255) / 256, 256, 0, stream>>>(a, consts);
 
     a.voice_tiles = (a.voices + SIG_WAVE * vpt - 1) / (SIG_WAVE * vpt);
     const int64_t nwg = ((int64_t)a.voice_tiles * ((a.K + a.span - 1) / a.span) + 3) / 4;
     if (nwg > 0x7fffffffLL) return (int)hipErrorInvalidValue;
     if (sig_bus::tiles_sum_in_workgroup(a.voice_tiles) && tuning().tile_sum_kernel == 0) { bus.out = out; bus.out_ld = out_ld; }
+    if constexpr (!GROWS && !CROWS) {
+        if (bus.out && a.voice_tiles == 1 && vpt >= 8) {
+            if (vpt == 16) fused_steady_bus_kernel<16, C, false, false, true><<<(unsigned)nwg, 256, 0, stream>>>(a, bus);
+            else fused_steady_bus_kernel<8, C, false, false, true><<<(unsigned)nwg, 256, 0, stream>>>(a, bus);
+            return sig_launch_status();
+        }
+    }
     switch (vpt) {
         case 1: fused_steady_bus_kernel<1, C, GROWS, CROWS><<<(unsigned)nwg, 256, 0, stream>>>(a, bus); break;
         case 2: fused_steady_bus_kernel<2, C, GROWS, CROWS><<<(unsigned)nwg, 256, 0, stream>>>(a, bus); break;
@@ -1411,19 +1430,33 @@
     return 0;
 }
 
-extern "C" int sig_fused_voice_bus_plan(int osc_kind, int64_t position, int32_t voices, int32_t block_frames, int32_t nblocks,
-                                       int32_t context, int32_t* voices_per_lane, int32_t* blocks_per_lane,
-                                       int32_t* closed_form)
+extern "C" int sig_fused_voice_bus_plan_for(int osc_kind, int64_t position, int32_t voices, int32_t block_frames, int32_t nblocks,
+                                           int32_t context, int32_t slots_decayed, int32_t* voices_per_lane,
+                                           int32_t* blocks_per_lane, int32_t* closed_form)
 {
     SIG_CHECK_ARG(voices >= 0 && block_frames >= 0 && nblocks >= 0 && context >= 0 && position >= 0);
     SIG_CHECK_ARG(voices_per_lane && blocks_per_lane && closed_form);
     FusedArgs a{};
     a.position = position; a.N = block_frames; a.K = nblocks; a.ctx = context; a.voices = voices;
+    a.consts_ready = slots_decayed ? 2 : 0;
     const BusPlan p = plan_voice_bus(a, osc_kind);
     *voices_per_lane = p.vpt;
     *blocks_per_lane = p.span;
     *closed_form = p.steady;
     return 0;
+}
+
+extern "C" int sig_fused_voice_bus_plan(int osc_kind, int64_t position, int32_t voices, int32_t block_frames, int32_t nblocks,
+                                       int32_t context, int32_t* voices_per_lane, int32_t* blocks_per_lane,
+                                       int32_t* closed_form)
+{
+    return sig_fused_voice_bus_plan_for(osc_kind, position, voices, block_frames, nblocks, context, 1, voices_per_lane,
+                                        blocks_per_lane, closed_form);
+}
+
+extern "C" int sig_fused_steady_live_slots(int32_t voices_per_lane)
+{
+    return (voices_per_lane == 16) ? SIG_STEADY_LIVE16 : voices_per_lane;
 }
 
 extern "C" int sig_fused_set_tuning(int32_t voices_per_lane, int32_t blocks_per_lane, int32_t closed_form, int32_t scan)
diff --git a/signals_amd/csrc/sig_bus_tile.h b/signals_amd/csrc/sig_bus_tile.h
--- a/signals_amd/csrc/sig_bus_tile.h
+++ b/signals_amd/csrc/sig_bus_tile.h
@@ -41,16 +41,17 @@
     }
 };
 
-template <int C>
+template <int C, bool F32 = false>
 struct PipelinedTile {
     static constexpr int R = kPairs / C;
     double* tile; const double* col; double* slot; double* dstp;
     int lane, staged;
     int64_t first;
+    float* out; int64_t out_ld;
 
-    __device__ __forceinline__ PipelinedTile(double* tile_, int lane_, double* dstp_, int64_t first_row)
+    __device__ __forceinline__ PipelinedTile(double* tile_, int lane_, double* dstp_, int64_t first_row, float* out_ = nullptr, int64_t out_ld_ = 0)
         : tile(tile_), col(tile_ + (lane_ & (kPairs - 1)) * kTileStride + (lane_ >> 4) * 16), slot(tile_ + lane_),
-          dstp(dstp_), lane(lane_), staged(0), first(first_row) {}
+          dstp(dstp_), lane(lane_), staged(0), first(first_row), out(out_), out_ld(out_ld_) {}
 
     __device__ __forceinline__ void issue(double (&pv)[16]) const {
 #pragma unroll
@@ -58,7 +59,8 @@
     }
     __device__ __forceinline__ void finish(const double (&pv)[16], int64_t row0, int nrows) const {
         const double s = sig_sum_rows_f64(sum16(pv));
-        if (lane < nrows * C) dstp[row0 * C + lane] = s;
+        if constexpr (F32) { if (lane < nrows * C) out[(row0 + lane / C) * out_ld + lane % C] = (float)(0.0 + s); }
+        else if (lane < nrows * C) dstp[row0 * C + lane] = s;
     }
     __device__ __forceinline__ void now() {
         double pv[16];
@@ -77,12 +79,13 @@
 
 constexpr int kFoldStride = 17;
 
-template <int C>
+template <int C, bool F32 = false>
 struct FoldedGroup {
     double* put; const double* get; double* dstp; int lane;
-    __device__ __forceinline__ FoldedGroup(double* tile, int lane_, double* dstp_)
+    float* out; int64_t out_ld;
+    __device__ __forceinline__ FoldedGroup(double* tile, int lane_, double* dstp_, float* out_ = nullptr, int64_t out_ld_ = 0)
         : put(tile + ((((lane_ >> 4) & 1) << 1) | (lane_ >> 5)) * kFoldStride + (lane_ & 15)),
-          get(tile + (lane_ & 15) * kFoldStride + 4 * (lane_ >> 4)), dstp(dstp_), lane(lane_) {}
+          get(tile + (lane_ & 15) * kFoldStride + 4 * (lane_ >> 4)), dstp(dstp_), lane(lane_), out(out_), out_ld(out_ld_) {}
     __device__ __forceinline__ void fold4(int q, double t0, double t1, double t2, double t3) const {
         put[4 * q * kFoldStride] = sig_fold16(sig_fold32(t0, t1), sig_fold32(t2, t3));
     }
@@ -92,7 +95,8 @@
     }
     __device__ __forceinline__ void finish(const double (&pv)[4], int64_t row0, int nrows) const {
         const double s = sig_sum_rows_f64((pv[0] + pv[1]) + (pv[2] + pv[3]));
-        if (lane < nrows * C) dstp[row0 * C + lane] = s;
+        if constexpr (F32) { if (lane < nrows * C) out[(row0 + lane / C) * out_ld + lane % C] = (float)(0.0 + s); }
+        else if (lane < nrows * C) dstp[row0 * C + lane] = s;
     }
 };
 
diff --git a/signals_amd/engine.py b/signals_amd/engine.py
--- a/signals_amd/engine.py
+++ b/signals_amd/engine.py
@@ -1226,6 +1226,21 @@
         pick = lambda t: t if t is None or t.shape[1] != v else t.index_select(1, index).contiguous()
         return [pick(t) for t in ctl], pick(pan)
 
+    def slots_decayed(self, ctl, voices_per_lane: int) -> bool:
+        import numpy as np
+        index, hz_src, cut_src = self.cutoff_order(ctl, voices_per_lane), self.src.hertz.sig, self.filt.cutoff.sig
+        if index is None or not isinstance(hz_src, fixed.Fixed) or not hz_src._state.enabled:
+            return False
+        hz = np.asarray(hz_src._state.value, dtype=np.float64).reshape(-1)
+        cut = np.asarray(cut_src._state.value, dtype=np.float64).reshape(-1)
+        if hz.size != cut.size:
+            if hz.size != 1:
+                return False
+            hz = np.full(cut.size, hz[0])
+        order = index.cpu().numpy()
+        return _native.steady_slots_decayed(_native.steady_decay_rows(self.btype, self.batch.rate, hz[order], cut[order]),
+                                            CONTEXT, voices_per_lane)
+
     def cutoff_order(self, ctl, voices_per_lane: int):
         import numpy as np
         v, src = self.channels, self.filt.cutoff.sig
@@ -1373,10 +1388,14 @@
                 size = _native.lib().sig_fused_voice_consts_size(v) // 8
                 buf = held[2] if held is not None and held[2].numel() >= size else torch.empty(size, dtype=CTRL_DTYPE, device=dev)
                 plan = _native.fused_voice_bus_plan(self.kind, position, v, N, K, CONTEXT)
-                o._steady_consts = held = (key, (tuple(ctl), pan_now), buf, self.cycles_per_frame_bound(),
+                vouch = plan['voices_per_lane'] == 16 and self.slots_decayed(ctl, 16)
+                if plan['voices_per_lane'] == 16 and not vouch:
+                    plan = _native.fused_voice_bus_plan(self.kind, position, v, N, K, CONTEXT, slots_decayed=False)
+                o._steady_consts = held = (key, (tuple(ctl), pan_now), buf, (*self.cycles_per_frame_bound(), 2 if vouch else 0),
                                            self.ordered_by_cutoff(ctl, pan_now, plan['voices_per_lane']))
             ctl, pan_now = held[4]
-            per_frame, ph_max = held[3]
+            ready = (1 if ready else 0) | held[3][2]
+            per_frame, ph_max = held[3][:2]
             walk = self.kind == 'Sine' and ph_max + (position + rows) * per_frame >= _native.SINE_FAST_MAX_CYCLES
             if o.timer is None or o.timer.region:
                 call = held[5] if len(held) > 5 else None
@@ -1442,7 +1461,7 @@
                     'outs': [[torch.empty((rows, bus_c), dtype=AUDIO_DTYPE, device=dev) for _ in range(RING)] for _ in streams],
                     'slot': [0] * len(streams)}
                 torch.cuda.synchronize()
-            per_frame, ph_max = held[3]
+            per_frame, ph_max = held[3][:2]
             if self.kind == 'Sine' and ph_max + (position + rows) * per_frame >= _native.SINE_FAST_MAX_CYCLES:
                 return None
             i = pipe['i']
@@ -1452,9 +1471,9 @@
             out = pipe['outs'][i][slot]
             call, handle = pipe['calls'][i], pipe['handles'][i]
             if o.timer is not None:
-                o.timer.launch(bus_name, lambda: call(position, out, True, False, stream=handle), units=rows * v)
+                o.timer.launch(bus_name, lambda: call(position, out, 1 | held[3][2], False, stream=handle), units=rows * v)
             else:
-                call(position, out, True, False, stream=handle)
+                call(position, out, 1 | held[3][2], False, stream=handle)
             pipe['events'][i].record(pipe['streams'][i])
             raw = _native.current_stream_handle(dev.index)
             cur = pipe.get('current')
```
